# Haian-Jin/TensoIR

Hardware: AMD Instinct MI355X
Metric: primary+secondary rays/sec at 4096 rays x 512 samples (higher is better)
Workload: dtype f32 io and field; decoders split-bf16 x3 (hi/lo operands, 3 MFMA products), fp32 accumulate; indirect light (secondary-ray records): fp16 shadow taps + fp16 single-product decoder, fp32 accumulate

## Files before the change

### include/tensoir_hip.h

```cpp
#ifndef TENSOIR_HIP_H
#define TENSOIR_HIP_H

#include <stdint.h>

#ifdef __cplusplus
extern "C" {
#endif

#define TIR_VERSION 100

#define TIR_OK               0
#define TIR_ERR_ARG         -1001
#define TIR_ERR_UNSUPPORTED -1002
#define TIR_ERR_NO_DEVICE   -1003

typedef struct TirField {
    float aabb_min[3];
    float aabb_max[3];
    float inv_aabb[3];
    int32_t grid[3];
    float step_size;
    float distance_scale;
    float density_shift;
    float weight_thres;
    float near_, far_;
    int32_t act;
    int32_t n_dcomp;
    int32_t n_acomp;
    int32_t app_dim;
    int32_t n_lights;
    const float* dplane[3];
    const float* dline[3];
    const float* aplane[3];
    const float* aline[3];
    const float* basis_t;
    const float* light_line;
    const float* light_mean;
    const uint8_t* occ_nbr;
    int32_t occ_dim[3];
    float occ_aabb_min[3];
    float occ_inv[3];
    float occ_lo[3];
    float occ_hi[3];
    int32_t tune_lds_lines;
    int32_t tune_xcd_order;
    const float* dense_sigma;
    int32_t dense_pitch;
} TirField;

typedef struct TirFieldHalf {
    const void* aplane[3];
    const void* aline[3];
} TirFieldHalf;

#define TIR_HALF_MAX_JOBS 8
typedef struct TirHalfJob { const float* src; void* dst; int64_t n; unsigned* absmax; } TirHalfJob;
typedef struct TirHalfJobs { TirHalfJob job[TIR_HALF_MAX_JOBS]; } TirHalfJobs;

typedef struct TirMlp {
    const float* packed;
    int32_t feat_dim;
    int32_t pe;
    int32_t hidden;
    int32_t out_dim;
    int32_t act;
    int32_t tune_grid;
} TirMlp;

typedef struct TirEnvSG {
    const float* sgs;
    const float* rot;
    int32_t n_sg;
    int32_t n_lights;
} TirEnvSG;

int  tir_version(void);
const char* tir_error_string(int code);
int  tir_device_check(void);

int tir_pack_plane(const float* src, float* dst, int32_t C, int32_t H, int32_t W, void* stream);
int tir_pack_occupancy(const float* vol, uint8_t* nbr, int32_t W, int32_t H, int32_t D, void* stream);
int tir_pack_basis(const float* w, float* dst, int32_t app_dim, int32_t n_in, void* stream);
int tir_light_mean(const float* light_line, float* mean, int32_t L, int32_t n, void* stream);
int64_t tir_mlp_packed_floats(int32_t feat_dim, int32_t pe, int32_t hidden, int32_t out_dim);
int tir_pack_mlp(const float* w0, const float* b0, const float* w1, const float* b1,
                 const float* w2, const float* b2, int32_t feat_dim, int32_t pe, int32_t hidden,
                 int32_t out_dim, float* packed, void* stream);

int tir_vm_density_fwd(const TirField* f, const float* xyz, float* feat, float* sigma,
                       int64_t n, void* stream);

int tir_occupancy_query(const TirField* f, const float* xyz, uint8_t* hit, int64_t n, void* stream);

int tir_dense_alpha(const TirField* f, const float* lin_x, const float* lin_y, const float* lin_z,
                    int32_t gx, int32_t gy, int32_t gz, float length, float* alpha, void* stream);
int tir_alpha_pool(const float* alpha, int32_t gx, int32_t gy, int32_t gz, float thres, float* vol,
                   int32_t* bbox, void* stream);
int tir_filter_rays(const TirField* f, const float* rays, int64_t n, int32_t n_samples, int32_t bbox_only,
                    uint8_t* mask, void* stream);

int tir_dense_sigma_build(const TirField* f, float* vol, int32_t pitch, void* stream);
int tir_dense_sigma_fwd(const TirField* f, const float* xyz, float* feat, float* sigma, int64_t n, void* stream);

int tir_density_grad_fwd(const TirField* f, const float* xyz, float* sigma, float* grad,
                         float* normal, int64_t n, const int32_t* n_dev, void* stream);
int tir_density_feat_grad_fwd(const TirField* f, const float* xyz, float* feat, float* grad, int64_t n, void* stream);

int tir_vm_app_fwd(const TirField* f, const float* xyz, const int32_t* light_idx,
                   const int32_t* idx_map, float* rad_feat, float* int_feat, int32_t out_stride,
                   int32_t idx_div, int64_t n, const int32_t* n_dev, void* stream);

int tir_vm_app_jitter_fwd(const TirField* f, const float* xyz, int64_t n, const int32_t* n_dev, float scale,
                          uint64_t seed, uint64_t offset, const int64_t* rng_state, float* xyz_out,
                          float* int_feat, int32_t out_stride, void* stream);

int tir_vm_app_primary_fwd(const TirField* f, const float* xyz, const int32_t* light_idx, const int32_t* idx_map,
                           float* rad_feat, float* int_feat, int32_t out_stride, int64_t n, const int32_t* n_dev,
                           float scale, uint64_t seed, uint64_t offset, const int64_t* rng_state, float* xyz_out,
                           float* int_feat_jit, void* stream);
int tir_vm_app_primary_x3_fwd(const TirField* f, const float* xyz, const int32_t* light_idx, const int32_t* idx_map,
                              float* rad_feat, float* int_feat, int32_t out_stride, int64_t n, const int32_t* n_dev,
                              float scale, uint64_t seed, uint64_t offset, const int64_t* rng_state, float* xyz_out,
                              float* int_feat_jit, void* stream);
int tir_vm_app_fwd_x3(const TirField* f, const float* xyz, const int32_t* light_idx,
                      const int32_t* idx_map, float* rad_feat, float* int_feat, int32_t out_stride,
                      int32_t idx_div, int64_t n, const int32_t* n_dev, void* stream);
int tir_vm_app_fwd_bf16x3(const TirField* f, const float* xyz, const int32_t* light_idx,
                          const int32_t* idx_map, float* rad_feat, float* int_feat, int32_t out_stride,
                          int32_t idx_div, int64_t n, const int32_t* n_dev, void* stream);
int tir_vm_app_fwd_valu(const TirField* f, const float* xyz, const int32_t* light_idx,
                        const int32_t* idx_map, float* rad_feat, float* int_feat, int32_t out_stride,
                        int32_t idx_div, int64_t n, const int32_t* n_dev, void* stream);

int tir_mlp_fwd(const TirMlp* m, const float* feat, int32_t feat_stride, const float* aux,
                const int32_t* aux_map, int32_t aux_mod, float* out, int64_t n, const int32_t* n_dev,
        void* stream);
int tir_mlp_fwd_bf16x3(const TirMlp* m, const float* feat, int32_t feat_stride, const float* aux,
                       const int32_t* aux_map, int32_t aux_mod, float* out, int64_t n, const int32_t* n_dev,
        void* stream);

int tir_pack_half(const float* const* srcs, void* const* dsts, const int64_t* counts, int32_t n_tables, void* stream);
int tir_pack_half_checked(const float* const* srcs, void* const* dsts, const int64_t* counts, int32_t n_tables, float* absmax,
                          void* stream);
int tir_vm_app_fwd_h16(const TirField* f, const TirFieldHalf* fh, const float* xyz, const int32_t* light_idx,
                       const int32_t* idx_map, float* rad_feat, int32_t out_stride, int32_t idx_div, int64_t n,
                       const int32_t* n_dev, void* stream);

int tir_indirect_fused_fwd(const TirField* f, const TirFieldHalf* fh, const TirMlp* m, const float* xyz,
                           const int32_t* light_idx, const int32_t* rec_map, int32_t idx_div, int32_t aux_mod,
                           const float* table, float* out, int64_t n, const int32_t* n_dev, void* stream);

int tir_indirect_fused_hp_fwd(const TirField* f, const TirMlp* m, const float* xyz, const int32_t* light_idx,
                              const int32_t* rec_map, int32_t idx_div, int32_t aux_mod, const float* table, float* out,
                              int64_t n, const int32_t* n_dev, void* stream);

int tir_mlp_fwd_multi_bf16x3(const TirMlp* const* mlps, const float* const* feats, int32_t feat_stride,
                             const float* const* auxs, const int32_t* const* aux_maps, float* const* outs,
                             int32_t n_jobs, int64_t n, const int32_t* n_dev, void* stream);

int tir_mlp_aux_table(const TirMlp* m, const float* aux, int64_t n_aux, float* table, void* stream);
int tir_mlp_fwd_auxtab_bf16x3(const TirMlp* m, const float* feat, int32_t feat_stride, const float* table,
                              const int32_t* aux_map, int32_t aux_mod, float* out, int64_t n, const int32_t* n_dev,
                              void* stream);
int tir_mlp_fwd_auxtab_f16(const TirMlp* m, const float* feat, int32_t feat_stride, const float* table,
                           const int32_t* aux_map, int32_t aux_mod, float* out, int64_t n, const int32_t* n_dev,
                           void* stream);
int tir_mlp_train_fwd_auxtab_bf16x3(const TirMlp* m, const float* feat, int32_t feat_stride, const float* table,
                                    const int32_t* aux_map, int32_t aux_mod, float* out, float* h1, float* h2, int64_t n,
                                    const int32_t* n_dev, void* stream);
int tir_mlp_fwd_multi_auxtab_bf16x3(const TirMlp* const* mlps, const float* const* feats, int32_t feat_stride,
                                    const float* const* auxs, const int32_t* const* aux_maps,
                                    const float* const* tables, float* const* outs, int32_t n_jobs, int64_t n,
                                    const int32_t* n_dev, void* stream);
int tir_mlp_train_fwd_multi_bf16x3(const TirMlp* const* mlps, const float* const* feats, int32_t feat_stride,
                                   const float* const* auxs, const int32_t* const* aux_maps, float* const* outs,
                                   float* const* h1s, float* const* h2s, int32_t n_jobs, int64_t n,
                                   const int32_t* n_dev, void* stream);
int tir_mlp_fwd_bf16(const TirMlp* m, const float* feat, int32_t feat_stride, const float* aux,
                     const int32_t* aux_map, int32_t aux_mod, float* out, int64_t n, const int32_t* n_dev,
        void* stream);
int tir_mlp_fwd_valu(const TirMlp* m, const float* feat, int32_t feat_stride, const float* aux,
                     const int32_t* aux_map, int32_t aux_mod, float* out, int64_t n, const int32_t* n_dev,
        void* stream);

int tir_march_primary_fwd(const TirField* f, const float* rays, const float* ray_jitter,
// ... 360 lines not shown
```

### tensoir_amd/_lib.py

```python
from __future__ import annotations

import ctypes as C
import os

_HERE = os.path.dirname(os.path.abspath(__file__))
LIB_PATH = os.environ.get("TENSOIR_HIP_LIB", os.path.join(_HERE, "libtensoir_hip.so"))

c_float_p = C.c_void_p
c_int_p = C.c_void_p


class TirField(C.Structure):
    _fields_ = [
        ("aabb_min", C.c_float * 3), ("aabb_max", C.c_float * 3), ("inv_aabb", C.c_float * 3),
        ("grid", C.c_int32 * 3),
        ("step_size", C.c_float), ("distance_scale", C.c_float), ("density_shift", C.c_float),
        ("weight_thres", C.c_float), ("near_", C.c_float), ("far_", C.c_float),
        ("act", C.c_int32), ("n_dcomp", C.c_int32), ("n_acomp", C.c_int32), ("app_dim", C.c_int32),
        ("n_lights", C.c_int32),
        ("dplane", C.c_void_p * 3), ("dline", C.c_void_p * 3),
        ("aplane", C.c_void_p * 3), ("aline", C.c_void_p * 3),
        ("basis_t", C.c_void_p), ("light_line", C.c_void_p), ("light_mean", C.c_void_p),
        ("occ_nbr", C.c_void_p),
        ("occ_dim", C.c_int32 * 3), ("occ_aabb_min", C.c_float * 3), ("occ_inv", C.c_float * 3),
        ("occ_lo", C.c_float * 3), ("occ_hi", C.c_float * 3),
        ("tune_lds_lines", C.c_int32), ("tune_xcd_order", C.c_int32),
        ("dense_sigma", C.c_void_p), ("dense_pitch", C.c_int32),
    ]


class TirFieldHalf(C.Structure):
    _fields_ = [("aplane", C.c_void_p * 3), ("aline", C.c_void_p * 3)]


class TirFieldGrad(C.Structure):
    _fields_ = [("dplane", C.c_void_p * 3), ("dline", C.c_void_p * 3), ("aplane", C.c_void_p * 3),
                ("aline", C.c_void_p * 3), ("light_line", C.c_void_p), ("light_mean", C.c_void_p)]


class TirMlp(C.Structure):
    _fields_ = [("packed", C.c_void_p), ("feat_dim", C.c_int32), ("pe", C.c_int32),
                ("hidden", C.c_int32), ("out_dim", C.c_int32), ("act", C.c_int32), ("tune_grid", C.c_int32)]


class TirEnvSG(C.Structure):
    _fields_ = [("sgs", C.c_void_p), ("rot", C.c_void_p), ("n_sg", C.c_int32), ("n_lights", C.c_int32)]


P = C.c_void_p
I32 = C.c_int32
I64 = C.c_int64
F32 = C.c_float

SIGNATURES = {
    "tir_version": (C.c_int, []),
    "tir_error_string": (C.c_char_p, [C.c_int]),
    "tir_device_check": (C.c_int, []),
    "tir_pack_plane": (C.c_int, [P, P, I32, I32, I32, P]),
    "tir_pack_occupancy": (C.c_int, [P, P, I32, I32, I32, P]),
    "tir_pack_basis": (C.c_int, [P, P, I32, I32, P]),
    "tir_light_mean": (C.c_int, [P, P, I32, I32, P]),
    "tir_mlp_packed_floats": (I64, [I32, I32, I32, I32]),
    "tir_pack_mlp": (C.c_int, [P, P, P, P, P, P, I32, I32, I32, I32, P, P]),
    "tir_vm_density_fwd": (C.c_int, [C.POINTER(TirField), P, P, P, I64, P]),
    "tir_occupancy_query": (C.c_int, [C.POINTER(TirField), P, P, I64, P]),
    "tir_dense_alpha": (C.c_int, [C.POINTER(TirField), P, P, P, I32, I32, I32, F32, P, P]),
    "tir_alpha_pool": (C.c_int, [P, I32, I32, I32, F32, P, P, P]),
    "tir_filter_rays": (C.c_int, [C.POINTER(TirField), P, I64, I32, I32, P, P]),
    "tir_dense_sigma_build": (C.c_int, [C.POINTER(TirField), P, I32, P]),
    "tir_dense_sigma_fwd": (C.c_int, [C.POINTER(TirField), P, P, P, I64, P]),
    "tir_density_grad_fwd": (C.c_int, [C.POINTER(TirField), P, P, P, P, I64, P, P]),
    "tir_density_feat_grad_fwd": (C.c_int, [C.POINTER(TirField), P, P, P, I64, P]),
    "tir_vm_app_fwd": (C.c_int, [C.POINTER(TirField), P, P, P, P, P, I32, I32, I64, P, P]),
    "tir_vm_app_fwd_bf16x3": (C.c_int, [C.POINTER(TirField), P, P, P, P, P, I32, I32, I64, P, P]),
    "tir_vm_app_fwd_x3": (C.c_int, [C.POINTER(TirField), P, P, P, P, P, I32, I32, I64, P, P]),
    "tir_pack_half": (C.c_int, [P, P, P, I32, P]),
    "tir_pack_half_checked": (C.c_int, [P, P, P, I32, P, P]),
    "tir_vm_app_fwd_h16": (C.c_int, [C.POINTER(TirField), C.POINTER(TirFieldHalf), P, P, P, P, I32, I32, I64, P, P]),
    "tir_indirect_fused_fwd": (C.c_int, [C.POINTER(TirField), C.POINTER(TirFieldHalf), C.POINTER(TirMlp), P, P, P, I32, I32, P, P, I64, P, P]),
    "tir_indirect_fused_hp_fwd": (C.c_int, [C.POINTER(TirField), C.POINTER(TirMlp), P, P, P, I32, I32, P, P, I64, P, P]),
    "tir_vm_app_fwd_valu": (C.c_int, [C.POINTER(TirField), P, P, P, P, P, I32, I32, I64, P, P]),
    "tir_mlp_fwd": (C.c_int, [C.POINTER(TirMlp), P, I32, P, P, I32, P, I64, P, P]),
    "tir_mlp_fwd_bf16x3": (C.c_int, [C.POINTER(TirMlp), P, I32, P, P, I32, P, I64, P, P]),
    "tir_mlp_fwd_multi_bf16x3": (C.c_int, [P, P, I32, P, P, P, I32, I64, P, P]),
    "tir_mlp_fwd_multi_auxtab_bf16x3": (C.c_int, [P, P, I32, P, P, P, P, I32, I64, P, P]),
    "tir_mlp_aux_table": (C.c_int, [C.POINTER(TirMlp), P, I64, P, P]),
    "tir_mlp_fwd_auxtab_bf16x3": (C.c_int, [C.POINTER(TirMlp), P, I32, P, P, I32, P, I64, P, P]),
    "tir_mlp_fwd_auxtab_f16": (C.c_int, [C.POINTER(TirMlp), P, I32, P, P, I32, P, I64, P, P]),
    "tir_mlp_train_fwd_auxtab_bf16x3": (C.c_int, [C.POINTER(TirMlp), P, I32, P, P, I32, P, P, P, I64, P, P]),
    "tir_mlp_train_fwd_multi_bf16x3": (C.c_int, [P, P, I32, P, P, P, P, P, I32, I64, P, P]),
    "tir_mlp_fwd_bf16": (C.c_int, [C.POINTER(TirMlp), P, I32, P, P, I32, P, I64, P, P]),
    "tir_mlp_fwd_valu": (C.c_int, [C.POINTER(TirMlp), P, I32, P, P, I32, P, I64, P, P]),
    "tir_march_primary_fwd": (C.c_int, [C.POINTER(TirField), P, P, I32, I32, F32, P, P, P, P, P, P, P]),
    "tir_exclusive_scan": (C.c_int, [P, P, I32, P]),
    "tir_exclusive_scan_capped": (C.c_int, [P, P, I32, I32, P, P]),
    "tir_march_primary_fused_fwd": (C.c_int, [C.POINTER(TirField), P, P, I32, I32, F32, P, P, P, P, P, P,
                                              P, P, I32, P, P, I32, P, P]),
    "tir_composite_primary_fused": (C.c_int, [P, P, P, P, P, P, P, P, P, P, I32, I32, I32, F32, P, P, P, P, I64, P]),
    "tir_vm_app_jitter_fwd": (C.c_int, [C.POINTER(TirField), P, I64, P, F32, C.c_uint64, C.c_uint64, P, P, P, I32, P]),
    "tir_vm_app_primary_fwd": (C.c_int, [C.POINTER(TirField), P, P, P, P, P, I32, I64, P, F32, C.c_uint64, C.c_uint64, P, P, P, P]),
    "tir_vm_app_primary_x3_fwd": (C.c_int, [C.POINTER(TirField), P, P, P, P, P, I32, I64, P, F32, C.c_uint64, C.c_uint64, P, P, P, P]),
    "tir_compact_primary": (C.c_int, [C.POINTER(TirField), P, P, P, P, I32, I32, P, P, P, P, P]),
    "tir_composite_primary": (C.c_int, [P, P, P, P, P, P, P, P, P, P, I32, I32, I32, F32, P, P]),
    "tir_march_secondary_fwd": (C.c_int, [C.POINTER(TirField), P, P, P, P, P, I64, I32, I32, P, F32, P, P,
                                          P, I64, P, P, P, P, P, P, P]),
    "tir_accumulate_records": (C.c_int, [P, P, P, P, I64, P, P]),
    "tir_env_sg_fwd": (C.c_int, [C.POINTER(TirEnvSG), P, I32, P, P]),
    "tir_env_pixel_fwd": (C.c_int, [P, I32, I32, P, P, I32, I64, I32, P, P]),
    "tir_env_pixel_bwd": (C.c_int, [P, I32, I32, P, P, I32, I64, P, P, P]),
    "tir_shade_setup": (C.c_int, [P, P, P, I32, I32, F32, P, P, P]),
    "tir_shade_integrate": (C.c_int, [P, P, P, P, P, P, P, P, I32, I32, I32, I32, I32, F32, P, P]),
    "tir_shade_integrate_records": (C.c_int, [P, P, P, P, P, P, P, P, P, P, P, I32, I32, I32, I32, I32, F32, P, P, P]),
    "tir_shade_setup_compact": (C.c_int, [P, P, P, I32, I32, F32, P, P, P, P, P, P, I32, P]),
    "tir_march_secondary_ids_fwd": (C.c_int, [C.POINTER(TirField), P, P, P, P, P, I64, I32, I32, P, F32, P, P,
                                              P, I64, P, P, P, P, P, P, P, P, P]),
    "tir_relight_importance": (C.c_int, [P, P, P, P, P, P, P, P, P, I32, I32, P, P]),
    "tir_env_sample_setup": (C.c_int, [P, P, I32, I32, P, P, I32, I32, C.c_uint64, C.c_uint64, P, P, P]),
    "tir_env_sample_setup_list": (C.c_int, [P, P, I32, I32, P, I32, P, I32, I32, C.c_uint64, C.c_uint64, I32, I32, I32, P, P, I32, I32, P, P, P, P, P]),
    "tir_relight_importance_cells": (C.c_int, [P, P, P, P, P, P, P, P, P, P, I32, I32, P, P]),
    "tir_relight_importance_cells_packed": (C.c_int, [P, P, P, P, P, P, P, P, I32, I32, P, P]),
    "tir_env_lookup": (C.c_int, [P, I32, I32, P, I64, P, P]),
    "tir_surface_compact": (C.c_int, [P, P, I32, C.c_float, P, P, P, P, P, P, P, P, P]),
    "tir_env_sample_setup_list_n": (C.c_int, [P, P, I32, I32, P, I32, P, I32, I32, C.c_uint64, C.c_uint64, I32, I32, I32, P, P, I32, I32, P, P, P, P, P, P]),
    "tir_relight_importance_cells_packed_n": (C.c_int, [P, P, P, P, P, P, P, P, I32, I32, P, P, P]),
    "tir_env_compose": (C.c_int, [P, I32, I32, P, I32, I64, P, P, P, I32, P]),
    "tir_env_mis_setup": (C.c_int, [P, P, I32, I32, P, I32, P, P, P, P, P, I32, I32, I32, F32, C.c_uint64, C.c_uint64, I32, P, P, I32, I32,
                                    P, P, P, P, P, P, P, P]),
    "tir_relight_mis": (C.c_int, [P, P, P, P, P, P, P, P, P, P, I32, I32, I32, P, P, P]),
    "tir_ggx_specular": (C.c_int, [P, P, P, P, P, I32, I32, P, P]),
    "tir_march_primary_train_fwd": (C.c_int, [C.POINTER(TirField), P, P, I32, I32, F32, P, P, P, P, P, P, P]),
    "tir_composite_primary_bwd": (C.c_int, [P] * 11 + [I32, I32, I32, I32, F32] + [P] * 9 + [P]),
    "tir_march_primary_bwd": (C.c_int, [C.POINTER(TirField), C.POINTER(TirFieldGrad), P, P, I32, I32, P, P, P, P, P, P, P]),
    "tir_density_grad_bwd": (C.c_int, [C.POINTER(TirField), C.POINTER(TirFieldGrad), P, P, I64, P]),
    "tir_vm_density_bwd": (C.c_int, [C.POINTER(TirField), C.POINTER(TirFieldGrad), P, P, I64, P]),
    "tir_density_feat_bwd": (C.c_int, [C.POINTER(TirField), C.POINTER(TirFieldGrad), P, P, P, I64, P]),
    "tir_density_feat_grad_bwd": (C.c_int, [C.POINTER(TirField), C.POINTER(TirFieldGrad), P, P, P, I64, P]),
    "tir_vm_app_bwd": (C.c_int, [C.POINTER(TirField), C.POINTER(TirFieldGrad), P, P, P, P, P, I32, I64, P, P, P]),
    "tir_mlp_train_fwd": (C.c_int, [C.POINTER(TirMlp), P, I32, P, P, I32, P, P, P, I64, P, P]),
    "tir_mlp_train_fwd_bf16x3": (C.c_int, [C.POINTER(TirMlp), P, I32, P, P, I32, P, P, P, I64, P, P]),
    "tir_mlp_inputs": (C.c_int, [C.POINTER(TirMlp), P, I32, P, P, I32, P, I64, P]),
    "tir_mlp_bwd_packed_floats": (I64, [I32, I32, I32, I32]),
    "tir_pack_mlp_bwd": (C.c_int, [P, P, P, I32, I32, I32, I32, P, P]),
    "tir_mlp_bwd": (C.c_int, [C.POINTER(TirMlp), P, P, I32, P, P, P, P, I64, P, P, P, P, P]),
    "tir_mlp_bwd_bf16x3": (C.c_int, [C.POINTER(TirMlp), P, P, I32, P, P, P, P, I64, P, P, P, P, P]),
    "tir_mlp_bwd_multi_bf16x3": (C.c_int, [P, P, P, I32, P, P, P, P, I32, I64, P, P, P, P, P]),
    "tir_gemm_tn_small_bf16x3": (C.c_int, [P, I32, I32, P, I32, I32, I32, I64, P, I32, P]),
    "tir_mlp_wgrad_multi": (C.c_int, [P, P, P, P, P, P, I32, P, P, P, P, P, P, P, P, I32, I64, I32, P]),
    "tir_record_check": (C.c_int, [P, P, I32, P, P, P]),
    "tir_adam_step": (C.c_int, [I32, P, P, P, P, P, P, P, P, F32, F32, F32, P]),
    "tir_gemm_tn": (C.c_int, [P, I32, I32, P, I32, I32, I32, I64, P, I32, P, P]),
    "tir_gemm_tn_bf16x3": (C.c_int, [P, I32, I32, P, I32, I32, I32, I64, P, I32, P, P]),
    "tir_shade_integrate_bwd": (C.c_int, [P, P, P, P, P, P, P, P, I32, I32, I32, I32, I32, F32, P, P, P, P]),
    "tir_env_sg_bwd": (C.c_int, [C.POINTER(TirEnvSG), P, I32, P, P, P]),
# ... 73 lines not shown
```

### tensoir_amd/csrc/tir_common.hpp

```cpp
#pragma once
#include <hip/hip_runtime.h>
#include <stdint.h>
#include <initializer_list>
#include <type_traits>
#include "tensoir_hip.h"

#define TIR_WAVE 64

#define TIR_CHECK_LAUNCH()                                   \
    do {                                                     \
        hipError_t e__ = hipGetLastError();                  \
        if (e__ != hipSuccess) return -(int)e__;             \
    } while (0)

static inline hipStream_t tir_stream(void* s) { return reinterpret_cast<hipStream_t>(s); }

static inline int tir_xcd_mapping(const TirField* f) { return f->tune_xcd_order == 1 ? 1 : 0; }

#include <mutex>
#include <set>
#include <utility>
static inline int tir_allow_dynamic_lds(const void* kernel, int bytes) {
    static std::mutex mu;
    static std::set<std::pair<const void*, int>> done;
    int dev = 0;
    hipError_t e = hipGetDevice(&dev);
    if (e != hipSuccess) return -(int)e;
    std::lock_guard<std::mutex> lock(mu);
    if (done.count({kernel, dev})) return TIR_OK;
    e = hipFuncSetAttribute(kernel, hipFuncAttributeMaxDynamicSharedMemorySize, bytes);
    if (e != hipSuccess) return -(int)e;
    done.insert({kernel, dev});
    return TIR_OK;
}

static inline bool tir_occ_index_ok(const TirField* f) {
    if (!f->occ_nbr) return true;
    const int64_t W = f->occ_dim[0], H = f->occ_dim[1], D = f->occ_dim[2];
    return W > 0 && H > 0 && D > 0 && W + 1 < (1 << 24) && (H + 1) * (D + 1) < (1 << 24) && (W + 1) * (H + 1) * (D + 1) < ((int64_t)1 << 31);
}

static inline bool tir_plane_index_ok(const TirField* f) {
    for (int i = 0; i < 3; ++i)
        for (int j = i + 1; j < 3; ++j)
            if ((int64_t)f->grid[i] * f->grid[j] * f->n_dcomp * 4 >= ((int64_t)1 << 32) || (int64_t)f->grid[i] * f->n_dcomp * 4 >= (1 << 24) || (int64_t)f->grid[j] * f->n_dcomp * 4 >= (1 << 24)) return false;
    return true;
}

static inline bool tir_app_index_ok(const TirField* f) {
    for (int i = 0; i < 3; ++i)
        for (int j = i + 1; j < 3; ++j)
            if ((int64_t)f->grid[i] * f->grid[j] * f->n_acomp >= ((int64_t)1 << 31)) return false;
    for (int i = 0; i < 3; ++i)
        if ((int64_t)f->grid[i] * f->n_acomp >= (1 << 24)) return false;
    return true;
}

static inline bool tir_dense_sigma_ok(const TirField* f) {
    if (!f->dense_sigma || f->dense_pitch <= f->grid[0]) return false;
    const int64_t Y = f->grid[1], Z = f->grid[2], pb = (int64_t)f->dense_pitch * 4;
    return f->grid[0] >= 2 && Y >= 1 && Z >= 1 && Y * Z < (1 << 24) && pb < (1 << 24) && Y * Z * pb < ((int64_t)1 << 32);
}

static inline bool tir_any_null(std::initializer_list<const void*> ptrs) {
    for (const void* p : ptrs) if (!p) return true;
    return false;
}
static inline bool tir_aligned16(std::initializer_list<const void*> ptrs) {
    for (const void* p : ptrs) if (reinterpret_cast<uintptr_t>(p) % 16 != 0) return false;
    return true;
}

struct TirAppNeeds {
    const TirFieldHalf* half = nullptr;
    bool aligned16 = false;
    bool light_mean = true;
    bool index32 = false;
    int n_acomp = 0;
    int app_dim = 0;
    bool feature_rows = true;
    int stride_max = 32;
    TirAppNeeds& fp16_tables(const TirFieldHalf* fh) { half = fh; return *this; }
    TirAppNeeds& aligned() { aligned16 = true; return *this; }
    TirAppNeeds& no_light_mean() { light_mean = false; return *this; }
    TirAppNeeds& element_index32() { index32 = true; return *this; }
    TirAppNeeds& width(int n) { n_acomp = n; return *this; }
    TirAppNeeds& app_dim_is(int d) { app_dim = d; return *this; }
    TirAppNeeds& no_feature_rows() { feature_rows = false; return *this; }
    TirAppNeeds& stride_unbounded() { stride_max = 0x7fffffff; return *this; }
};

static inline int tir_check_app_field(const TirField* f, const TirAppNeeds& need, int out_stride) {
    for (int i = 0; i < 3; ++i) {
        const void* plane = need.half ? need.half->aplane[i] : static_cast<const void*>(f->aplane[i]);
        const void* line = need.half ? need.half->aline[i] : static_cast<const void*>(f->aline[i]);
        if (f->grid[i] < 2 || !plane || !line || (need.aligned16 && !tir_aligned16({plane, line}))) return TIR_ERR_ARG;
    }
    if (!f->basis_t || !f->light_line || (need.light_mean && !f->light_mean)) return TIR_ERR_ARG;
    if (need.n_acomp && f->n_acomp != need.n_acomp) return TIR_ERR_UNSUPPORTED;
    if (need.app_dim ? f->app_dim != need.app_dim : (f->app_dim < 1 || f->app_dim > 27)) return TIR_ERR_UNSUPPORTED;
    if (need.index32 && !tir_app_index_ok(f)) return TIR_ERR_UNSUPPORTED;
    if (need.feature_rows && (out_stride < f->app_dim || out_stride > need.stride_max)) return TIR_ERR_ARG;
    return TIR_OK;
}

template <typename Go>
static inline int tir_with_rows(int64_t n, std::initializer_list<const void*> need, std::initializer_list<const void*> aligned, Go&& go) {
    if (n < 0 || (n > 0 && tir_any_null(need)) || !tir_aligned16(aligned)) return TIR_ERR_ARG;
    if (n == 0) return TIR_OK;
    return go();
}

constexpr int TIR_APP_LDS_LIMIT = 160 * 1024;

static inline unsigned tir_gather_blocks(int64_t n, int rows, int cap, int xcd_on) {
    int64_t blocks = (n + rows - 1) / rows;
    if (blocks > cap) blocks = cap;
    if (xcd_on) blocks = (blocks + 7) / 8 * 8;
    return (unsigned)blocks;
}

static inline unsigned tir_job_split(int64_t units, int total, int n_jobs) {
    int per = total / n_jobs;
    if (per < 1) per = 1;
    if (units < per) per = (int)units;
    return (unsigned)(per * n_jobs);
}

template <typename... P, typename... A>
static inline int tir_launch(void (*kernel)(P...), int lds_limit, dim3 grid, dim3 block, size_t lds, hipStream_t s, const A&... args) {
    if (lds_limit > 0)
        if (int rc = tir_allow_dynamic_lds(reinterpret_cast<const void*>(kernel), lds_limit)) return rc;
    hipLaunchKernelGGL(kernel, grid, block, lds, s, args...);
    TIR_CHECK_LAUNCH();
    return TIR_OK;
}

template <int... C4S, typename Fn>
static inline int tir_dispatch_c4(int n_acomp, Fn&& fn) {
    int rc = TIR_ERR_UNSUPPORTED;
    (void)((n_acomp == 4 * C4S && ((rc = fn(std::integral_constant<int, C4S>{})), true)) || ...);
    return rc;
}

// ... 354 lines not shown
__device__ __forceinline__ float scan_prod(float v, int ) {
    v *= dpp_f<0x111, 0xf>(1.0f, v);
    v *= dpp_f<0x112, 0xf>(1.0f, v);
    v *= dpp_f<0x114, 0xf>(1.0f, v);
    v *= dpp_f<0x118, 0xf>(1.0f, v);
    v *= dpp_f<0x142, 0xa>(1.0f, v);
    if (WIDTH == 64) v *= dpp_f<0x143, 0xc>(1.0f, v);
    return v;
}

template <int WIDTH>
__device__ __forceinline__ float shift_up1(float incl, int lane_in_group) {
    float o = dpp_f<0x138, 0xf>(1.0f, incl);
    return lane_in_group == 0 ? 1.0f : o;
}

template <int WIDTH>
__device__ __forceinline__ float group_sum(float v) {
#pragma unroll
    for (int d = WIDTH / 2; d > 0; d >>= 1) v += __shfl_xor(v, d, WIDTH);
    return v;
}

template <int C4>
__device__ __forceinline__ float wave_sigma_t(const TirField& f, bool valid, float x, float y, float z, float* wl) {
    const int lane = threadIdx.x & 63;
    const unsigned long long m = __ballot(valid);
    const int n = __popcll(m);
    if (n == 0) return 0.0f;
    const int rank = __popcll(m & ((1ull << lane) - 1ull));
    if (valid) { wl[rank * 4] = x; wl[rank * 4 + 1] = y; wl[rank * 4 + 2] = z; }
    __builtin_amdgcn_wave_barrier();
    constexpr int PER = 64 / C4;
    const int slot_in = lane / C4, c = lane % C4;
    for (int base = 0; base < n; base += PER) {
        const int slot = base + slot_in;
        float part = 0.0f;
        if (slot < n) {
            const float4 p = *reinterpret_cast<const float4*>(wl + slot * 4);
            part = density_feature_chunk<C4>(f, p.x, p.y, p.z, c);
        }
        if (C4 >= 2) part += dpp_f<0xB1, 0xf>(0.0f, part);
        if (C4 >= 4) part += dpp_f<0x4E, 0xf>(0.0f, part);
        if (C4 >= 8) part += dpp_f<0x141, 0xf>(0.0f, part);
        if (slot < n && c == 0) wl[slot * 4 + 3] = part;
    }
    __builtin_amdgcn_wave_barrier();
    float sig = 0.0f;
    if (valid) sig = feature2density(f, wl[rank * 4 + 3]);
    __builtin_amdgcn_wave_barrier();
    return sig;
}

#define TIR_TAPREC 9

__device__ __forceinline__ unsigned mad_u24(unsigned a, unsigned b, unsigned c) {
    unsigned r;
    asm("v_mad_u32_u24 %0, %1, %2, %3" : "=v"(r) : "v"(a), "v"(b), "v"(c));
    return r;
}

typedef float tir_f2u __attribute__((ext_vector_type(2), aligned(4)));

__device__ __forceinline__ tir_f2 ld2b(const float* base, unsigned byte_off) {
    const tir_f2u v = *reinterpret_cast<const tir_f2u*>(reinterpret_cast<const char*>(base) + byte_off);
    return tir_f2{v.x, v.y};
}

__device__ __forceinline__ float dense_feature(const TirField& f, float x, float y, float z) {
    const TapQ tx = make_tap_q(x, f.grid[0]), ty = make_tap_q(y, f.grid[1]), tz = make_tap_q(z, f.grid[2]);
    const bool below = tx.i1 == 0u;
    const float wx0 = below ? tx.w.y : tx.w.x, wx1 = below ? 0.0f : tx.w.y;
    const unsigned pb = (unsigned)f.dense_pitch * 4u, xo = tx.i0 * 4u;
    const unsigned z0 = mul_u24(tz.i0, (unsigned)f.grid[1]), z1 = mul_u24(tz.i1, (unsigned)f.grid[1]);
    const tir_f2 v00 = ld2b(f.dense_sigma, mad_u24(z0 + ty.i0, pb, xo));
    const tir_f2 v01 = ld2b(f.dense_sigma, mad_u24(z0 + ty.i1, pb, xo));
    const tir_f2 v10 = ld2b(f.dense_sigma, mad_u24(z1 + ty.i0, pb, xo));
    const tir_f2 v11 = ld2b(f.dense_sigma, mad_u24(z1 + ty.i1, pb, xo));
    const float a = fmaf(v00.y, wx1, v00.x * wx0), b = fmaf(v01.y, wx1, v01.x * wx0);
    const float c = fmaf(v10.y, wx1, v10.x * wx0), d = fmaf(v11.y, wx1, v11.x * wx0);
    const float e = fmaf(b, ty.w.y, a * ty.w.x), g = fmaf(d, ty.w.y, c * ty.w.x);
    return fmaf(g, tz.w.y, e * tz.w.x);
}
__device__ __forceinline__ unsigned lds_addr(const float* p) {
#if defined(__HIP_DEVICE_COMPILE__)
    return (unsigned)(uintptr_t)(const __attribute__((address_space(3))) float*)p;
#else
    return 0;
#endif
}
__device__ __forceinline__ float4 lds_ld4(unsigned addr) {
#if defined(__HIP_DEVICE_COMPILE__)
    return *(const __attribute__((address_space(3))) float4*)(uintptr_t)addr;
#else
    return float4{};
#endif
}

template <int C4>
__device__ __forceinline__ float density_chunk_rec(const TirField& f, const float* __restrict__ ll, const unsigned* __restrict__ rec, int c) {
    constexpr unsigned TB = C4 * 16;
    const unsigned pk[3] = {rec[0], rec[1], rec[2]};
    unsigned ix[3][2];
#pragma unroll
    for (int a = 0; a < 3; ++a) { ix[a][0] = pk[a] & 0xffffu; ix[a][1] = pk[a] >> 16; }
    const unsigned cb = 16u * (unsigned)c;
    unsigned col[2][2];
#pragma unroll
    for (int a = 0; a < 2; ++a) { col[a][0] = mad_u24(ix[a][0], TB, cb); col[a][1] = mad_u24(ix[a][1], TB, cb); }
    float acc = 0.0f;
    unsigned laddr = lds_addr(ll) + cb;
#pragma unroll
    for (int i = 0; i < 3; ++i) {
        const int m0 = (i == 2) ? 1 : 0, m1 = (i == 0) ? 1 : 2, vi = 2 - i;
        const unsigned row_bytes = (unsigned)f.grid[m0] * TB;
        const float* pl = f.dplane[i];
        const float4 a = ld4b(pl, mad_u24(ix[m1][0], row_bytes, col[m0][0]));
        const float4 b = ld4b(pl, mad_u24(ix[m1][0], row_bytes, col[m0][1]));
        const float4 cc = ld4b(pl, mad_u24(ix[m1][1], row_bytes, col[m0][0]));
        const float4 d = ld4b(pl, mad_u24(ix[m1][1], row_bytes, col[m0][1]));
        const float4 e = lds_ld4(mad_u24(ix[vi][0], TB, laddr));
        const float4 g = lds_ld4(mad_u24(ix[vi][1], TB, laddr));
        laddr += (unsigned)f.grid[vi] * TB;
        const tir_f2 w0 = {__uint_as_float(rec[3 + 2 * m0]), __uint_as_float(rec[4 + 2 * m0])};
        const tir_f2 w1 = {__uint_as_float(rec[3 + 2 * m1]), __uint_as_float(rec[4 + 2 * m1])};
        const tir_f2 wv = {__uint_as_float(rec[3 + 2 * vi]), __uint_as_float(rec[4 + 2 * vi])};
        const tir_f2 wa = w0 * tir_f2{w1.x, w1.x}, wb = w0 * tir_f2{w1.y, w1.y};
        acc = plane_line_4ch(a, b, cc, d, e, g, wa, wb, wv, acc);
    }
    return acc;
}

template <int C4>
__device__ __forceinline__ float wave_sigma_lds(const TirField& f, const float* __restrict__ ll, bool valid, float x, float y,
                                                float z, float* wl) {
    const int lane = threadIdx.x & 63;
    const unsigned long long m = __ballot(valid);
    const int n = __popcll(m);
    if (n == 0) return 0.0f;
    const int rank = __popcll(m & ((1ull << lane) - 1ull));
    unsigned* const wr = reinterpret_cast<unsigned*>(wl);
    if (valid) {
        const TapQ tx = make_tap_q(x, f.grid[0]), ty = make_tap_q(y, f.grid[1]), tz = make_tap_q(z, f.grid[2]);
        unsigned* r = wr + rank * TIR_TAPREC;
        r[0] = tx.i0 | (tx.i1 << 16); r[1] = ty.i0 | (ty.i1 << 16); r[2] = tz.i0 | (tz.i1 << 16);
        r[3] = __float_as_uint(tx.w.x); r[4] = __float_as_uint(tx.w.y);
        r[5] = __float_as_uint(ty.w.x); r[6] = __float_as_uint(ty.w.y);
        r[7] = __float_as_uint(tz.w.x); r[8] = __float_as_uint(tz.w.y);
    }
    __builtin_amdgcn_wave_barrier();
    constexpr int PER = 64 / C4;
    const int slot_in = lane / C4, c = lane % C4;
    for (int base = 0; base < n; base += PER) {
        const int slot = base + slot_in;
        float part = 0.0f;
        if (slot < n) part = density_chunk_rec<C4>(f, ll, wr + slot * TIR_TAPREC, c);
        if (C4 >= 2) part += dpp_f<0xB1, 0xf>(0.0f, part);
        if (C4 >= 4) part += dpp_f<0x4E, 0xf>(0.0f, part);
        if (C4 >= 8) part += dpp_f<0x141, 0xf>(0.0f, part);
        if (slot < n && c == 0) wl[slot * TIR_TAPREC] = part;
    }
    __builtin_amdgcn_wave_barrier();
    float sig = 0.0f;
    if (valid) sig = feature2density(f, wl[rank * TIR_TAPREC]);
    __builtin_amdgcn_wave_barrier();
    return sig;
// ... 192 lines not shown
```

### tensoir_amd/csrc/tir_field.hip

```cpp
#include "tir_common.hpp"

using namespace tir;

__global__ void k_pack_plane(const float* __restrict__ src, float* __restrict__ dst, int C, int HW) {
    int64_t i = (int64_t)blockIdx.x * blockDim.x + threadIdx.x;
    if (i >= (int64_t)C * HW) return;
    int c = (int)(i % C);
    int64_t t = i / C;
    dst[i] = src[(int64_t)c * HW + t];
}

__global__ void k_pack_occ(const float* __restrict__ vol, uint8_t* __restrict__ nbr, int W, int H, int D) {
    int64_t i = (int64_t)blockIdx.x * blockDim.x + threadIdx.x;
    const int64_t n = (int64_t)(W + 1) * (H + 1) * (D + 1);
    if (i >= n) return;
    const int x0 = (int)(i % (W + 1)) - 1, y0 = (int)((i / (W + 1)) % (H + 1)) - 1, z0 = (int)(i / ((int64_t)(W + 1) * (H + 1))) - 1;
    uint32_t m = 0;
    for (int c = 0; c < 8; ++c) {
        const int xx = x0 + (c & 1), yy = y0 + ((c >> 1) & 1), zz = z0 + (c >> 2);
        if (xx >= 0 && xx < W && yy >= 0 && yy < H && zz >= 0 && zz < D && vol[((int64_t)zz * H + yy) * W + xx] > 0.5f) m |= 1u << c;
    }
    nbr[i] = (uint8_t)m;
}

// ... 1118 lines not shown
    return tir_with_rows(n, {xyz}, {}, [&] {
        constexpr int C4 = 12, CA = 48;
        const int lt_rows = f->n_lights <= 16 ? f->n_lights : 0;
        const size_t w_floats = HX ? (2 * 3 * 2 * 2 * 64 * 16) / 4 : 3 * CA * 32;
        const size_t x_floats = HX ? (2 * 2 * 16 * TIR_XHX * 2) / 4 : 2 * CA * TIR_XLD;
        const int nb = (int)tir_gather_blocks(n, 64, 1024, 1);
        const dim3 g(2 * nb), b(256);
        const int xcd_on = tir_xcd_mapping(f);
        const TirJitter jt{scale, (unsigned long long)seed, (unsigned long long)offset, reinterpret_cast<const long long*>(rng_state), xyz_out};
        if (f->n_lights == 1) {
            const size_t lds1 = (w_floats + (size_t)2 * 3 * CA + 4 * (x_floats / 2)) * sizeof(float);
            return tir_launch(k_vm_app_primary_one<C4, HX>, TIR_APP_LDS_LIMIT, g, b, lds1, tir_stream(stream), *f, xyz, rad_feat, int_feat,
                              int_feat_jit, out_stride, n, n_dev, xcd_on, jt, nb);
        }
        const size_t lds = (w_floats + (size_t)(lt_rows + 1) * 3 * CA + 4 * x_floats) * sizeof(float);
        return tir_launch(k_vm_app_primary<C4, HX>, TIR_APP_LDS_LIMIT, g, b, lds, tir_stream(stream), *f, xyz, light_idx, idx_map, rad_feat,
                          int_feat, int_feat_jit, out_stride, n, n_dev, xcd_on, jt, lt_rows, nb);
    });
}

extern "C" int tir_vm_app_primary_fwd(const TirField* f, const float* xyz, const int32_t* light_idx, const int32_t* idx_map,
                                      float* rad_feat, float* int_feat, int32_t out_stride, int64_t n, const int32_t* n_dev,
                                      float scale, uint64_t seed, uint64_t offset, const int64_t* rng_state, float* xyz_out,
                                      float* int_feat_jit, void* stream) {
    return app_primary_fwd<false>(f, xyz, light_idx, idx_map, rad_feat, int_feat, out_stride, n, n_dev, scale, seed, offset, rng_state,
                                  xyz_out, int_feat_jit, stream);
}

extern "C" int tir_vm_app_primary_x3_fwd(const TirField* f, const float* xyz, const int32_t* light_idx, const int32_t* idx_map,
                                         float* rad_feat, float* int_feat, int32_t out_stride, int64_t n, const int32_t* n_dev,
                                         float scale, uint64_t seed, uint64_t offset, const int64_t* rng_state, float* xyz_out,
                                         float* int_feat_jit, void* stream) {
    return app_primary_fwd<true>(f, xyz, light_idx, idx_map, rad_feat, int_feat, out_stride, n, n_dev, scale, seed, offset, rng_state,
                                 xyz_out, int_feat_jit, stream);
}

extern "C" int tir_vm_app_fwd_x3(const TirField* f, const float* xyz, const int32_t* light_idx,
                                 const int32_t* idx_map, float* rad_feat, float* int_feat, int32_t out_stride,
                                 int32_t idx_div, int64_t n, const int32_t* n_dev, void* stream) {
    return app_fwd(f, xyz, light_idx, idx_map, rad_feat, int_feat, out_stride, idx_div, n, n_dev, stream, APP_HX);
}

extern "C" int tir_vm_app_fwd_valu(const TirField* f, const float* xyz, const int32_t* light_idx,
                                   const int32_t* idx_map, float* rad_feat, float* int_feat, int32_t out_stride,
                                   int32_t idx_div, int64_t n, const int32_t* n_dev, void* stream) {
    return app_fwd(f, xyz, light_idx, idx_map, rad_feat, int_feat, out_stride, idx_div, n, n_dev, stream, APP_VALU);
}

extern "C" int tir_vm_app_fwd_bf16x3(const TirField* f, const float* xyz, const int32_t* light_idx,
                                     const int32_t* idx_map, float* rad_feat, float* int_feat, int32_t out_stride,
                                     int32_t idx_div, int64_t n, const int32_t* n_dev, void* stream) {
    return app_fwd(f, xyz, light_idx, idx_map, rad_feat, int_feat, out_stride, idx_div, n, n_dev, stream, APP_BF16X3);
}

static int pack_half_launch(const float* const* srcs, void* const* dsts, const int64_t* counts, int32_t n_tables, float* absmax, void* stream) {
    if (n_tables < 0 || n_tables > TIR_HALF_MAX_JOBS || (n_tables > 0 && (!srcs || !dsts || !counts))) return TIR_ERR_ARG;
    if (n_tables == 0) return TIR_OK;
    TirHalfJobs jobs;
    int64_t most = 0;
    for (int i = 0; i < n_tables; ++i) {
        if (counts[i] < 0 || (counts[i] > 0 && !srcs[i])) return TIR_ERR_ARG;
        if (counts[i] > 0 && !dsts[i] && !absmax) return TIR_ERR_ARG;
        if (reinterpret_cast<uintptr_t>(srcs[i]) % 16 != 0 || reinterpret_cast<uintptr_t>(dsts[i]) % 16 != 0) return TIR_ERR_ARG;
        jobs.job[i] = TirHalfJob{srcs[i], dsts[i], counts[i], absmax ? reinterpret_cast<unsigned*>(absmax) + i : nullptr};
        most = counts[i] > most ? counts[i] : most;
    }
    if (most == 0) return TIR_OK;
    const int64_t per_block = 2048 * TIR_PACK_CHUNKS;
    hipLaunchKernelGGL(k_pack_half, dim3((unsigned)((most + per_block - 1) / per_block), (unsigned)n_tables), dim3(256), 0, tir_stream(stream), jobs);
    TIR_CHECK_LAUNCH();
    return TIR_OK;
}

extern "C" int tir_pack_half(const float* const* srcs, void* const* dsts, const int64_t* counts, int32_t n_tables, void* stream) {
    return pack_half_launch(srcs, dsts, counts, n_tables, nullptr, stream);
}

extern "C" int tir_pack_half_checked(const float* const* srcs, void* const* dsts, const int64_t* counts, int32_t n_tables, float* absmax,
                                     void* stream) {
    if (!absmax) return TIR_ERR_ARG;
    return pack_half_launch(srcs, dsts, counts, n_tables, absmax, stream);
}

extern "C" int tir_vm_app_fwd_h16(const TirField* f, const TirFieldHalf* fh, const float* xyz, const int32_t* light_idx,
                                  const int32_t* idx_map, float* rad_feat, int32_t out_stride, int32_t idx_div, int64_t n,
                                  const int32_t* n_dev, void* stream) {
    if (!f || !fh) return TIR_ERR_ARG;
    if (int rc = tir_check_app_field(f, TirAppNeeds().fp16_tables(fh).aligned().element_index32().width(48), out_stride)) return rc;
    return tir_with_rows(n, {xyz, rad_feat, light_idx}, {}, [&] {
        const int lt_rows = f->n_lights <= 16 ? f->n_lights : 0;
        const size_t lds = (size_t)(3 * 3 * 2 * 32) * 16 + (size_t)(lt_rows + 1) * 144 * sizeof(float) + (size_t)4 * 32 * TIR_XH * 2;
        const int xcd_on = tir_xcd_mapping(f);
        return tir_launch(k_vm_app_h16, 0, dim3(tir_gather_blocks(n, 128, 2048, xcd_on)), dim3(256), lds, tir_stream(stream), *f, *fh, xyz,
                          light_idx, idx_map, rad_feat, out_stride, idx_div, n, n_dev, xcd_on, lt_rows);
    });
}
```

### tensoir_amd/csrc/tir_mlp.hip

```cpp
#include "tir_common.hpp"

typedef float f32x16 __attribute__((ext_vector_type(16)));
typedef float f32x4 __attribute__((ext_vector_type(4)));

namespace {

constexpr int F = 27;
constexpr int PE = 2;
constexpr int HID = 128;
constexpr int IN = F + 3 + 2 * PE * F + 2 * PE * 3;
constexpr int HALF = IN / 2;
constexpr int NPF = PE * F;
constexpr int R0 = HALF - NPF;

constexpr int OFF_W0 = 0;
constexpr int OFF_B0 = OFF_W0 + IN * HID;
constexpr int OFF_W1 = OFF_B0 + HID;
constexpr int OFF_B1 = OFF_W1 + HID * HID;
constexpr int OFF_W2 = OFF_B1 + HID;
constexpr int OFF_B2 = OFF_W2 + 2 * 64 * 4;
constexpr int MFMA_FLOATS = OFF_B2 + 4;
constexpr int OFF_RW0 = MFMA_FLOATS;
constexpr int OFF_RB0 = OFF_RW0 + HID * IN;
constexpr int OFF_RW1 = OFF_RB0 + HID;
// ... 659 lines not shown

__device__ __forceinline__ int fus_feature_of_row(int row) {
    const int kg = (row >> 2) & 1, slot = (row >> 3) * 4 + (row & 3);
    if (kg == 0) return slot < FUS_NF0 ? slot : -1;
    return slot < F - FUS_NF0 ? FUS_NF0 + slot : -1;
}

template <int KK>
__device__ __forceinline__ float fus_input(const float (&fo)[16]) {
    constexpr int j = KK / 5, kind = KK % 5;
    if constexpr (j >= FUS_NF0) return 0.0f;
    else if constexpr (kind == 4) return fo[j];
    else {
        const float c_hi = 0.15915493667125702f, c_lo = 6.4206382432985265e-09f;
        const float kr = rintf(fo[j] * c_hi);
        float t = fmaf(fo[j], c_hi, -kr);
        t = fmaf(fo[j], c_lo, t);
        const float sn = __builtin_amdgcn_sinf(t), cs = __builtin_amdgcn_sinf(t + 0.25f);
        if constexpr (kind == 0) return sn;
        else if constexpr (kind == 1) return (sn + sn) * cs;
        else if constexpr (kind == 2) return cs;
        else return fmaf(-(sn + sn), sn, 1.0f);
    }
}

template <int KB>
__device__ __forceinline__ void fus_layer1(unsigned whi, const float (&fo)[16], f32x16 (&acc)[4]) {
    bf16x8 ah[4], al[4];
#pragma unroll
    for (int mt = 0; mt < 4; ++mt) ah[mt] = lds_tile(whi, KB * 4096 + mt * 512);
    const float v[8] = {fus_input<KB * 8 + 0>(fo), fus_input<KB * 8 + 1>(fo), fus_input<KB * 8 + 2>(fo), fus_input<KB * 8 + 3>(fo),
                        fus_input<KB * 8 + 4>(fo), fus_input<KB * 8 + 5>(fo), fus_input<KB * 8 + 6>(fo), fus_input<KB * 8 + 7>(fo)};
    bf16x8 xh, xl = {};
    cvt8_f16(v, xh);
    mfma12<1, true>(ah, al, xh, xl, acc);
    __builtin_amdgcn_sched_barrier(0);
    if constexpr (KB + 1 < KB0A) fus_layer1<KB + 1>(whi, fo, acc);
}

typedef _Float16 fus_f16x2 __attribute__((ext_vector_type(2)));

template <int KB>
__device__ __forceinline__ void fus_layer2p(unsigned whi, const unsigned (&hp)[32], f32x16 (&acc)[4]) {
    bf16x8 ah[4], al[4];
#pragma unroll
    for (int mt = 0; mt < 4; ++mt) ah[mt] = lds_tile(whi, KB * 4096 + mt * 512);
    const u32x4_t H = {hp[4 * KB], hp[4 * KB + 1], hp[4 * KB + 2], hp[4 * KB + 3]};
    const bf16x8 xh = __builtin_bit_cast(bf16x8, H), xl = {};
    mfma12<1, true>(ah, al, xh, xl, acc);
    __builtin_amdgcn_sched_barrier(0);
    if constexpr (KB + 1 < KB1) fus_layer2p<KB + 1>(whi, hp, acc);
}

struct FusGroup { unsigned o00, o01, o10, o11, l0, l1; tir::tir_h2 w00, w01, w10, w11, wl0, wl1; };

__device__ __forceinline__ FusGroup fus_group(const TirField& f, const tir::TapQ (&ax)[3], const unsigned (&xb)[3][2], const int k) {
    constexpr int CA = 48;
    const int m0 = (k == 2) ? 1 : 0, m1 = (k == 0) ? 1 : 2, vi = 2 - k;
    const tir::TapQ &tx = ax[m0], &ty = ax[m1], &tl = ax[vi];
    FusGroup g;
    const float w00 = tx.w.x * ty.w.x, w01 = tx.w.y * ty.w.x, w10 = tx.w.x * ty.w.y, w11 = tx.w.y * ty.w.y;
    g.w00 = tir::tir_h2{(_Float16)w00, (_Float16)w00}; g.w01 = tir::tir_h2{(_Float16)w01, (_Float16)w01};
    g.w10 = tir::tir_h2{(_Float16)w10, (_Float16)w10}; g.w11 = tir::tir_h2{(_Float16)w11, (_Float16)w11};
    g.wl0 = tir::tir_h2{(_Float16)tl.w.x, (_Float16)tl.w.x}; g.wl1 = tir::tir_h2{(_Float16)tl.w.y, (_Float16)tl.w.y};
    const unsigned row_bytes = (unsigned)f.grid[m0] * (2 * CA);
    const unsigned r0 = tir::mul_u24(ty.i0, row_bytes), r1 = tir::mul_u24(ty.i1, row_bytes);
    g.o00 = r0 + xb[m0][0]; g.o01 = r0 + xb[m0][1]; g.o10 = r1 + xb[m0][0]; g.o11 = r1 + xb[m0][1];
    g.l0 = xb[vi][0]; g.l1 = xb[vi][1];
    return g;
}

struct FusChunk { uint4 a, b, c, d, e, g; };

__device__ __forceinline__ uint4 ld_u4b(const void* base, unsigned byte_off) {
    return *reinterpret_cast<const uint4*>(reinterpret_cast<const char*>(base) + byte_off);
}

__device__ __forceinline__ void fus_issue(FusChunk& c, const void* __restrict__ pl, const void* __restrict__ ln, const FusGroup& g, const int q) {
    const unsigned o = 32u * (unsigned)q;
    c.a = ld_u4b(pl, g.o00 + o); c.b = ld_u4b(pl, g.o01 + o); c.c = ld_u4b(pl, g.o10 + o); c.d = ld_u4b(pl, g.o11 + o);
    c.e = ld_u4b(ln, g.l0 + o);  c.g = ld_u4b(ln, g.l1 + o);
}

template <int NW, bool PACK>
__global__ void __launch_bounds__(NW * 64)
k_indirect_fused(TirField f, TirFieldHalf fh, const float* __restrict__ packed, const float* __restrict__ xyz,
                 const int32_t* __restrict__ light_idx, const int32_t* __restrict__ rec_map, int idx_div, int aux_mod,
                 const float* __restrict__ table, float* __restrict__ out, int64_t n, const int32_t* __restrict__ n_dev,
                 int out_dim, int act, int lt_rows) {
    using namespace tir;
    constexpr int CA = 48;
    extern __shared__ __attribute__((aligned(16))) float lds[];
    for (int i = threadIdx.x * 4; i < FH_FLOATS; i += NW * 64 * 4)
        *reinterpret_cast<float4*>(lds + i) = *reinterpret_cast<const float4*>(packed + OFF_FF + i);
    f16x8* Wh = reinterpret_cast<f16x8*>(lds + FH_FLOATS);
    float* LT = lds + FH_FLOATS + FUS_WH_BYTES / 4;
    const int n_lt = lt_rows;
    const int lane = threadIdx.x & 63, wave = threadIdx.x >> 6;
    _Float16* X = reinterpret_cast<_Float16*>(LT + (n_lt + 1) * (3 * CA)) + wave * (32 * FUS_XH);
    for (int e = threadIdx.x; e < 3 * 3 * 2 * 32; e += NW * 64) {
        const int row = e & 31, kg = (e >> 5) & 1, t = (e >> 6) % 3, k = e / 192;
        const int feat = fus_feature_of_row(row);
        f16x8 hv;
#pragma unroll
        for (int q = 0; q < 8; ++q) hv[q] = feat >= 0 ? sat_half(f.basis_t[(size_t)(k * CA + 16 * t + 8 * kg + q) * 32 + feat]) : (_Float16)0.0f;
        Wh[e] = hv;
    }
    _Float16* LT16 = reinterpret_cast<_Float16*>(LT);
    for (int i = threadIdx.x; i < n_lt * 3 * CA; i += NW * 64) LT16[i] = sat_half(f.light_line[i]);
    for (int i = threadIdx.x * 4; i < 3 * CA; i += NW * 64 * 4)
        *reinterpret_cast<float4*>(LT + n_lt * 3 * CA + i) = *reinterpret_cast<const float4*>(f.light_mean + i);
    __syncthreads();
    if (n_dev) n = min(n, (int64_t)max(*n_dev, 0));
    const int sl = lane & 31, h = lane >> 5;
    const int gj = lane >> 1, gc = lane & 1;
    const unsigned lds0 = (unsigned)(size_t)lds;
    const unsigned lane_off = lds0 + BH_FLOATS * 4 + (unsigned)(h * 128 + sl) * 16;
    const unsigned w0hi = opaque(lane_off);
    const unsigned w1hi = opaque(lane_off + BW0A_ELEMS * 2);
    constexpr int TILE = NW * 32;
    const int64_t n_tiles = (n + TILE - 1) / TILE;
    const UDiv by_div = make_udiv(idx_div), by_mod = make_udiv(aux_mod);
    for (int64_t tile = blockIdx.x; tile < n_tiles; tile += gridDim.x) {
        const int64_t r0 = tile * TILE + wave * 32;
        const int64_t sg = r0 + gj, sgc = sg < n ? sg : n - 1;
        const float p[3] = {xyz[3 * sgc], xyz[3 * sgc + 1], xyz[3 * sgc + 2]};
        const float* lrow;
        const _Float16* lrow16;
        {
            int li = 0;
            if (f.n_lights > 1) {
                unsigned lsel = rec_map ? (unsigned)rec_map[sgc] : (unsigned)sgc, rem_;
                lsel = udiv(lsel, by_div, rem_);
                li = light_idx[lsel];
                li = min(max(li, 0), f.n_lights - 1);
            }
            lrow = n_lt ? LT + li * (3 * CA) : f.light_line + (size_t)li * (3 * CA);
            lrow16 = LT16 + li * (3 * CA);
        }
        const int64_t sd = r0 + sl, sdc = sd < n ? sd : n - 1;
        unsigned ai = rec_map ? (unsigned)rec_map[sdc] : (unsigned)sdc;
        if (aux_mod > 0) udiv(ai, by_mod, ai);
        f32x16 facc;
#pragma unroll
        for (int r = 0; r < 16; ++r) facc[r] = 0.0f;
        f32x16 acc[4];
        auto load_table = [&]() {
            const float* tp = table + (size_t)ai * HID + 4 * h;
#pragma unroll
            for (int mt = 0; mt < 4; ++mt)
#pragma unroll
                for (int i = 0; i < 4; ++i) {
                    const float4 t4 = *reinterpret_cast<const float4*>(tp + mt * 32 + 8 * i);
                    acc[mt][4 * i] = t4.x; acc[mt][4 * i + 1] = t4.y; acc[mt][4 * i + 2] = t4.z; acc[mt][4 * i + 3] = t4.w;
                }
        };
        {
            TapQ ax[3];
            unsigned xb[3][2];
#pragma unroll
            for (int a = 0; a < 3; ++a) {
                ax[a] = make_tap_q(p[a], f.grid[a]);
                xb[a][0] = mul_u24(ax[a].i0, 2 * CA) + 16u * (unsigned)gc;
                xb[a][1] = mul_u24(ax[a].i1, 2 * CA) + 16u * (unsigned)gc;
            }
            FusGroup G[3];
            FusChunk ck[3];
            G[0] = fus_group(f, ax, xb, 0);
            fus_issue(ck[0], fh.aplane[0], fh.aline[0], G[0], 0);
            fus_issue(ck[1], fh.aplane[0], fh.aline[0], G[0], 1);
            fus_issue(ck[2], fh.aplane[0], fh.aline[0], G[0], 2);
#pragma unroll
            for (int i = 0; i < 9; ++i) {
                const int k = i / 3, q = i % 3;
                FusChunk& c = ck[i % 3];
                const int ch0 = 16 * q + 8 * gc;
                *reinterpret_cast<uint4*>(X + gj * FUS_XH + ch0) =
                    h16_chunk_pk(c.a, c.b, c.c, c.d, c.e, c.g, G[k].w00, G[k].w01, G[k].w10, G[k].w11, G[k].wl0, G[k].wl1,
                                 n_lt ? *reinterpret_cast<const uint4*>(lrow16 + k * CA + ch0) : pack8_half(lrow + k * CA + ch0));
                if (i + 3 < 9) {
                    const int k2 = (i + 3) / 3, q2 = (i + 3) % 3;
                    if (q2 == 0) G[k2] = fus_group(f, ax, xb, k2);
                    fus_issue(c, fh.aplane[k2], fh.aline[k2], G[k2], q2);
                }
                __builtin_amdgcn_wave_barrier();
                const f16x8 a = Wh[((k * 3 + q) * 2 + h) * 32 + sl];
                const f16x8 b = *reinterpret_cast<const f16x8*>(X + sl * FUS_XH + 16 * q + 8 * h);
                facc = __builtin_amdgcn_mfma_f32_32x32x16_f16(a, b, facc, 0, 0, 0);
                __builtin_amdgcn_wave_barrier();
            }
        }
        __builtin_amdgcn_s_setprio(FUS_DECODER_PRIO);
        float fo[16];
#pragma unroll
        for (int r = 0; r < 16; ++r) fo[r] = __builtin_amdgcn_fmed3f(facc[r], -65504.0f, 65504.0f);
        if (PACK) load_table();
        fus_layer1<0>(w0hi, fo, acc);
        f32x16 acc2[4];
        if constexpr (PACK) {
            unsigned hp[32];
#pragma unroll
            for (int q = 0; q < 64; q += 2) {
                const f32x2_t v2 = {acc[q >> 4][q & 15], acc[(q + 1) >> 4][(q + 1) & 15]};
                fus_f16x2 hv = __builtin_convertvector(v2, fus_f16x2);
                hv = __builtin_elementwise_min(__builtin_elementwise_max(hv, fus_f16x2{(_Float16)0.0f, (_Float16)0.0f}),
                                               fus_f16x2{(_Float16)65504.0f, (_Float16)65504.0f});
                hp[q >> 1] = __builtin_bit_cast(unsigned, hv);
            }
#pragma unroll
            for (int mt = 0; mt < 4; ++mt) {
                const float* bp = lds + BH_B1 + (h * 4 + mt) * 16;
#pragma unroll
                for (int r = 0; r < 16; ++r) acc2[mt][r] = bp[r];
            }
            fus_layer2p<0>(w1hi, hp, acc2);
        } else {
#pragma unroll
            for (int mt = 0; mt < 4; ++mt) {
                const float* bp = lds + BH_B1 + (h * 4 + mt) * 16;
#pragma unroll
                for (int r = 0; r < 16; ++r) acc2[mt][r] = bp[r];
            }
            layer2_interleaved<1, 0, true>(w1hi, w1hi, acc, acc2);
        }
        f32x4 o4[4];
#pragma unroll
        for (int c = 0; c < 4; ++c) o4[c] = f32x4{0.f, 0.f, 0.f, 0.f};
        {
            const float* wp = lds + BH_W2 + (h * 4 + (lane & 3)) * W2A_STRIDE;
#pragma unroll
            for (int g = 0; g < 16; ++g) {
                const float4 w = *reinterpret_cast<const float4*>(wp + 4 * g);
                const float wv[4] = {w.x, w.y, w.z, w.w};
#pragma unroll
                for (int e = 0; e < 4; ++e) {
                    const int q = 4 * g + e;
                    const float x = acc2[q >> 4][q & 15];
                    o4[e] = __builtin_amdgcn_mfma_f32_4x4x1f32(wv[e], x + __builtin_fabsf(x), o4[e], 0, 0, 0);
                }
            }
        }
        float o0 = (o4[0][0] + o4[1][0]) + (o4[2][0] + o4[3][0]);
        float o1 = (o4[0][1] + o4[1][1]) + (o4[2][1] + o4[3][1]);
        float o2 = (o4[0][2] + o4[1][2]) + (o4[2][2] + o4[3][2]);
        float o3 = (o4[0][3] + o4[1][3]) + (o4[2][3] + o4[3][3]);
        o0 += __shfl_xor(o0, 32, 64); o1 += __shfl_xor(o1, 32, 64);
        o2 += __shfl_xor(o2, 32, 64); o3 += __shfl_xor(o3, 32, 64);
        __builtin_amdgcn_s_setprio(0);
        if (h == 0 && sd < n) {
            const float* b2 = lds + BH_B2;
            float* op = out + sd * out_dim;
            op[0] = act_out(o0 + b2[0], act);
            if (out_dim > 1) op[1] = act_out(o1 + b2[1], act);
            if (out_dim > 2) op[2] = act_out(o2 + b2[2], act);
            if (out_dim > 3) op[3] = act_out(o3 + b2[3], act);
        }
    }
}

constexpr int HP_XS = 24;
constexpr int HP_X_HALVES = 2 * 32 * HP_XS;

typedef __attribute__((address_space(3))) const long lds_i64;
__device__ __forceinline__ long lds_tile8(unsigned base, int byte_off) {
    return *reinterpret_cast<lds_i64*>(base + (unsigned)byte_off);
}

__device__ __forceinline__ long cvt8_fp8(const float (&c)[8]) {
    int lo = 0, hi = 0;
    lo = __builtin_amdgcn_cvt_pk_fp8_f32(c[0], c[1], lo, false);
    lo = __builtin_amdgcn_cvt_pk_fp8_f32(c[2], c[3], lo, true);
    hi = __builtin_amdgcn_cvt_pk_fp8_f32(c[4], c[5], hi, false);
    hi = __builtin_amdgcn_cvt_pk_fp8_f32(c[6], c[7], hi, true);
    return (long)(((unsigned long)(unsigned)hi << 32) | (unsigned long)(unsigned)lo);
}

template <int KK>
__device__ __forceinline__ float fus_input8(const float (&fo)[16], const float (&fo8)[16]) {
    if constexpr (KK % 5 == 4 && KK / 5 < FUS_NF0) return fo8[KK / 5];
    else return fus_input<KK>(fo);
}

typedef int hp_i32x8 __attribute__((ext_vector_type(8)));
typedef __attribute__((address_space(3))) const u32x4_t lds_u32x4;

__device__ __forceinline__ void hp_residue(unsigned w8, int byte_off, const hp_i32x8& xs, f32x16 (&acc)[4]) {
#pragma unroll
    for (int mt = 0; mt < 4; ++mt) {
        const u32x4_t lo = *reinterpret_cast<lds_u32x4*>(w8 + (unsigned)(byte_off + mt * 1024));
        const u32x4_t hi = *reinterpret_cast<lds_u32x4*>(w8 + (unsigned)(byte_off + mt * 1024 + 16));
        const hp_i32x8 a = {(int)lo[0], (int)lo[1], (int)lo[2], (int)lo[3], (int)hi[0], (int)hi[1], (int)hi[2], (int)hi[3]};
        acc[mt] = __builtin_amdgcn_mfma_scale_f32_32x32x64_f8f6f4(a, xs, acc[mt], 0, 0, 0, 110, 0, 127);
    }
}

template <int KB>
__device__ __forceinline__ void hp_layer1(unsigned whi, unsigned w8, const float (&fo)[16], const float (&fo8)[16], f32x16 (&acc)[4],
                                          hp_i32x8& xs) {
    bf16x8 ah[4];
#pragma unroll
    for (int mt = 0; mt < 4; ++mt) ah[mt] = lds_tile(whi, KB * 4096 + mt * 512);
    const float v[8] = {fus_input<KB * 8 + 0>(fo), fus_input<KB * 8 + 1>(fo), fus_input<KB * 8 + 2>(fo), fus_input<KB * 8 + 3>(fo),
                        fus_input<KB * 8 + 4>(fo), fus_input<KB * 8 + 5>(fo), fus_input<KB * 8 + 6>(fo), fus_input<KB * 8 + 7>(fo)};
    const float v8[8] = {fus_input8<KB * 8 + 0>(fo, fo8), fus_input8<KB * 8 + 1>(fo, fo8), fus_input8<KB * 8 + 2>(fo, fo8), fus_input8<KB * 8 + 3>(fo, fo8),
                         fus_input8<KB * 8 + 4>(fo, fo8), fus_input8<KB * 8 + 5>(fo, fo8), fus_input8<KB * 8 + 6>(fo, fo8), fus_input8<KB * 8 + 7>(fo, fo8)};
    bf16x8 xh;
    cvt8_f16(v, xh);
    const long x8 = cvt8_fp8(v8);
    if constexpr (KB % 4 == 0) xs = hp_i32x8{0, 0, 0, 0, 0, 0, 0, 0};
    xs[2 * (KB % 4)] = (int)(unsigned)(unsigned long)x8;
    xs[2 * (KB % 4) + 1] = (int)(unsigned)((unsigned long)x8 >> 32);
#pragma unroll
    for (int mt = 0; mt < 4; ++mt)
        acc[mt] = __builtin_amdgcn_mfma_f32_32x32x16_f16(__builtin_bit_cast(f16x8, ah[mt]), __builtin_bit_cast(f16x8, xh), acc[mt], 0, 0, 0);
    if constexpr (KB % 4 == 3 || KB + 1 == KB0A) hp_residue(w8, (KB / 4) * 8192, xs, acc);
    __builtin_amdgcn_sched_barrier(0);
    if constexpr (KB + 1 < KB0A) hp_layer1<KB + 1>(whi, w8, fo, fo8, acc, xs);
}

template <int KB>
__device__ __forceinline__ void hp_layer2(unsigned whi, unsigned w8, const unsigned (&hp)[32], const unsigned (&h8)[16], f32x16 (&acc)[4]) {
    bf16x8 ah[4];
#pragma unroll
    for (int mt = 0; mt < 4; ++mt) ah[mt] = lds_tile(whi, KB * 4096 + mt * 512);
    const u32x4_t H = {hp[4 * KB], hp[4 * KB + 1], hp[4 * KB + 2], hp[4 * KB + 3]};
#pragma unroll
    for (int mt = 0; mt < 4; ++mt)
        acc[mt] = __builtin_amdgcn_mfma_f32_32x32x16_f16(__builtin_bit_cast(f16x8, ah[mt]), __builtin_bit_cast(f16x8, H), acc[mt], 0, 0, 0);
    if constexpr (KB % 4 == 3) {
        constexpr int g = KB / 4;
        const hp_i32x8 xs = {(int)h8[8 * g], (int)h8[8 * g + 1], (int)h8[8 * g + 2], (int)h8[8 * g + 3],
                             (int)h8[8 * g + 4], (int)h8[8 * g + 5], (int)h8[8 * g + 6], (int)h8[8 * g + 7]};
        hp_residue(w8, g * 8192, xs, acc);
    }
    __builtin_amdgcn_sched_barrier(0);
    if constexpr (KB + 1 < KB1) hp_layer2<KB + 1>(whi, w8, hp, h8, acc);
}

constexpr unsigned HP_TB = 192;
// ... 1252 lines not shown
        if (SAVE && n > 0 && (!h1s[i] || !h2s[i])) return TIR_ERR_ARG;
        if (!tir_aligned16({feats[i], tab})) return TIR_ERR_ARG;
        jobs.j[i] = TirMlpJob{mlps[i]->packed, feats[i], auxs[i], aux_maps ? aux_maps[i] : nullptr, outs[i], mlps[i]->out_dim,
                              mlps[i]->act, SAVE ? h1s[i] : nullptr, SAVE ? h2s[i] : nullptr, tab};
    }
    if (n == 0) return TIR_OK;
    return tir_launch(k_mlp_bf16_multi<3, SAVE>, BF_BYTES, dim3(tir_job_split((n + 255) / 256, 256, n_jobs)), dim3(512), (size_t)BF_BYTES,
                      tir_stream(stream), jobs, feat_stride, n, n_dev);
}

extern "C" int tir_mlp_fwd_multi_bf16x3(const TirMlp* const* mlps, const float* const* feats, int32_t feat_stride,
                                        const float* const* auxs, const int32_t* const* aux_maps, float* const* outs,
                                        int32_t n_jobs, int64_t n, const int32_t* n_dev, void* stream) {
    return launch_multi<false>(mlps, feats, feat_stride, auxs, aux_maps, outs, nullptr, nullptr, n_jobs, n, n_dev, stream);
}

extern "C" int tir_mlp_fwd_multi_auxtab_bf16x3(const TirMlp* const* mlps, const float* const* feats, int32_t feat_stride,
                                               const float* const* auxs, const int32_t* const* aux_maps,
                                               const float* const* tables, float* const* outs, int32_t n_jobs, int64_t n,
                                               const int32_t* n_dev, void* stream) {
    return launch_multi<false>(mlps, feats, feat_stride, auxs, aux_maps, outs, nullptr, nullptr, n_jobs, n, n_dev, stream, tables);
}

extern "C" int tir_mlp_train_fwd_multi_bf16x3(const TirMlp* const* mlps, const float* const* feats, int32_t feat_stride,
                                              const float* const* auxs, const int32_t* const* aux_maps, float* const* outs,
                                              float* const* h1s, float* const* h2s, int32_t n_jobs, int64_t n,
                                              const int32_t* n_dev, void* stream) {
    return launch_multi<true>(mlps, feats, feat_stride, auxs, aux_maps, outs, h1s, h2s, n_jobs, n, n_dev, stream);
}

extern "C" int tir_mlp_aux_table(const TirMlp* m, const float* aux, int64_t n_aux, float* table, void* stream) {
    if (int rc = check_mlp(m)) return rc;
    return tir_with_rows(n_aux, {aux, table}, {}, [&] {
        return tir_launch(k_mlp_aux_table, 0, dim3((unsigned)((n_aux * HID + 255) / 256)), dim3(256), 0, tir_stream(stream), m->packed, aux,
                          n_aux, table);
    });
}

#define TIR_AUXT_ARGS m->packed, feat, feat_stride, table, aux_map, aux_mod, out, n, n_dev, m->out_dim, m->act
template <bool F16, bool SAVE>
static int mlp_fwd_auxtab(const TirMlp* m, const float* feat, int32_t feat_stride, const float* table, const int32_t* aux_map,
                          int32_t aux_mod, float* out, float* h1, float* h2, int64_t n, const int32_t* n_dev, void* stream) {
    const auto go = [&] {
        const bool vec = rows_vec(feat, feat_stride);
        const dim3 g(decoder_grid(n, 256, m->tune_grid)), b(512);
        hipStream_t s = tir_stream(stream);
        if constexpr (F16)
            return vec ? tir_launch(k_mlp_f16_auxt<true>, FH_BYTES, g, b, FH_BYTES, s, TIR_AUXT_ARGS)
                       : tir_launch(k_mlp_f16_auxt<false>, FH_BYTES, g, b, FH_BYTES, s, TIR_AUXT_ARGS);
        else
            return vec ? tir_launch(k_mlp_bf16_auxt<true, SAVE>, BFA_BYTES, g, b, BFA_BYTES, s, TIR_AUXT_ARGS, h1, h2)
                       : tir_launch(k_mlp_bf16_auxt<false, SAVE>, BFA_BYTES, g, b, BFA_BYTES, s, TIR_AUXT_ARGS, h1, h2);
    };
    if constexpr (SAVE) return with_decoder_rows(m, n, feat_stride, {}, {feat, table, out, h1, h2}, {table}, go);
    else return with_decoder_rows(m, n, feat_stride, {}, {feat, table, out}, {table}, go);
}

#undef TIR_AUXT_ARGS

extern "C" int tir_mlp_fwd_auxtab_bf16x3(const TirMlp* m, const float* feat, int32_t feat_stride, const float* table,
                                         const int32_t* aux_map, int32_t aux_mod, float* out, int64_t n, const int32_t* n_dev,
                                         void* stream) {
    return mlp_fwd_auxtab<false, false>(m, feat, feat_stride, table, aux_map, aux_mod, out, nullptr, nullptr, n, n_dev, stream);
}

extern "C" int tir_mlp_fwd_auxtab_f16(const TirMlp* m, const float* feat, int32_t feat_stride, const float* table,
                                      const int32_t* aux_map, int32_t aux_mod, float* out, int64_t n, const int32_t* n_dev,
                                      void* stream) {
    return mlp_fwd_auxtab<true, false>(m, feat, feat_stride, table, aux_map, aux_mod, out, nullptr, nullptr, n, n_dev, stream);
}

extern "C" int tir_mlp_train_fwd_auxtab_bf16x3(const TirMlp* m, const float* feat, int32_t feat_stride, const float* table,
                                               const int32_t* aux_map, int32_t aux_mod, float* out, float* h1, float* h2,
                                               int64_t n, const int32_t* n_dev, void* stream) {
    return mlp_fwd_auxtab<false, true>(m, feat, feat_stride, table, aux_map, aux_mod, out, h1, h2, n, n_dev, stream);
}

extern "C" int tir_indirect_fused_fwd(const TirField* f, const TirFieldHalf* fh, const TirMlp* m, const float* xyz,
                                      const int32_t* light_idx, const int32_t* rec_map, int32_t idx_div, int32_t aux_mod,
                                      const float* table, float* out, int64_t n, const int32_t* n_dev, void* stream) {
    if (!f || !fh) return TIR_ERR_ARG;
    if (int rc = check_mlp(m)) return rc;
    if (int rc = tir_check_app_field(f, TirAppNeeds().fp16_tables(fh).aligned().element_index32().width(48).app_dim_is(F).no_feature_rows(), 0)) return rc;
    return tir_with_rows(n, {xyz, light_idx, table, out}, {table}, [&] {
        if (!fused_index_ok(n, idx_div, aux_mod)) return (int)TIR_ERR_UNSUPPORTED;
        const int lt_rows = f->n_lights <= 16 ? f->n_lights : 0;
        constexpr int NW = 12; constexpr bool PACK = true;
        const size_t lds = (size_t)FH_BYTES + FUS_WH_BYTES + (size_t)(lt_rows + 1) * 144 * sizeof(float) + (size_t)NW * 32 * FUS_XH * 2;
        return tir_launch(k_indirect_fused<NW, PACK>, (int)lds, dim3(decoder_grid(n, NW * 32, m->tune_grid)), dim3(NW * 64), lds,
                          tir_stream(stream), *f, *fh, m->packed, xyz, light_idx, rec_map, idx_div, aux_mod, table, out, n, n_dev,
                          m->out_dim, m->act, lt_rows);
    });
}

extern "C" int tir_indirect_fused_hp_fwd(const TirField* f, const TirMlp* m, const float* xyz, const int32_t* light_idx,
                                         const int32_t* rec_map, int32_t idx_div, int32_t aux_mod, const float* table, float* out,
                                         int64_t n, const int32_t* n_dev, void* stream) {
    if (!f) return TIR_ERR_ARG;
    if (int rc = check_mlp(m)) return rc;
    if (int rc = tir_check_app_field(f, TirAppNeeds().aligned().no_light_mean().element_index32().width(48).app_dim_is(F).no_feature_rows(), 0)) return rc;
    for (int i = 0; i < 3; ++i)
        for (int j = i + 1; j < 3; ++j)
            if ((int64_t)f->grid[i] * HP_TB >= (1 << 24) || (int64_t)f->grid[j] * HP_TB >= (1 << 24) ||
                (int64_t)f->grid[i] * f->grid[j] * HP_TB >= ((int64_t)1 << 32)) return TIR_ERR_UNSUPPORTED;
    return tir_with_rows(n, {xyz, light_idx, table, out}, {table}, [&] {
        if (!fused_index_ok(n, idx_div, aux_mod)) return (int)TIR_ERR_UNSUPPORTED;
        if (f->n_lights < 1 || f->n_lights > 8) return (int)TIR_ERR_UNSUPPORTED;
        const int lt_rows = f->n_lights;
        constexpr int NW = 8;
        const size_t lds = (size_t)FH_BYTES + (size_t)F8_FLOATS * 4 + 2 * (size_t)FUS_WH_BYTES + (size_t)lt_rows * 144 * sizeof(float) +
                           (size_t)NW * HP_X_HALVES * 2;
        return tir_launch(k_indirect_fused_hp<NW>, (int)lds, dim3(decoder_grid(n, NW * 32, m->tune_grid)), dim3(NW * 64), lds,
                          tir_stream(stream), *f, m->packed, xyz, light_idx, rec_map, idx_div, aux_mod, table, out, n, n_dev, m->out_dim,
                          m->act, lt_rows);
    });
}

extern "C" int64_t tir_mlp_bwd_packed_floats(int32_t feat_dim, int32_t pe, int32_t hidden, int32_t out_dim) {
    return mlp_shape_built(feat_dim, pe, hidden, out_dim) ? (int64_t)BWD_TOTAL_FLOATS : (int64_t)TIR_ERR_UNSUPPORTED;
}

extern "C" int tir_pack_mlp_bwd(const float* w0, const float* w1, const float* w2, int32_t feat_dim, int32_t pe,
                                int32_t hidden, int32_t out_dim, float* packed, void* stream) {
    if (tir_any_null({w0, w1, w2, packed})) return TIR_ERR_ARG;
    if (!mlp_shape_built(feat_dim, pe, hidden, out_dim)) return TIR_ERR_UNSUPPORTED;
    return tir_launch(k_pack_mlp_bwd, 0, dim3((BWD_TOTAL_FLOATS + 255) / 256), dim3(256), 0, tir_stream(stream), w0, w1, w2, out_dim, packed);
}

template <typename Kernel>
static int mlp_bwd(Kernel kernel, size_t lds, const TirMlp* m, const float* packed_bwd, const float* feat, int32_t feat_stride,
                   const float* out, const float* g_out, const float* h1, const float* h2, int64_t n, float* g_feat, float* dz1,
                   float* dz2, float* dz3, void* stream) {
    return with_decoder_rows(m, n, feat_stride, {packed_bwd}, {feat, out, g_out, h1, h2, g_feat, dz1, dz2, dz3}, {}, [&] {
        return tir_launch(kernel, (int)lds, dim3(decoder_grid(n, 256, NO_TUNE_GRID)), dim3(512), lds, tir_stream(stream), packed_bwd, feat,
                          feat_stride, out, g_out, h1, h2, n, m->out_dim, m->act, g_feat, dz1, dz2, dz3);
    });
}

extern "C" int tir_mlp_bwd(const TirMlp* m, const float* packed_bwd, const float* feat, int32_t feat_stride,
                           const float* out, const float* g_out, const float* h1, const float* h2, int64_t n,
                           float* g_feat, float* dz1, float* dz2, float* dz3, void* stream) {
    return mlp_bwd(k_mlp_bwd, (size_t)BWD_FLOATS * sizeof(float), m, packed_bwd, feat, feat_stride, out, g_out, h1, h2, n, g_feat, dz1, dz2,
                   dz3, stream);
}

extern "C" int tir_mlp_bwd_bf16x3(const TirMlp* m, const float* packed_bwd, const float* feat, int32_t feat_stride,
                           const float* out, const float* g_out, const float* h1, const float* h2, int64_t n,
                           float* g_feat, float* dz1, float* dz2, float* dz3, void* stream) {
    return mlp_bwd(k_mlp_bwd_bf16, (size_t)BWD_BF_LDS_BYTES, m, packed_bwd, feat, feat_stride, out, g_out, h1, h2, n, g_feat, dz1, dz2, dz3,
                   stream);
}

extern "C" int tir_mlp_bwd_multi_bf16x3(const TirMlp* const* mlps, const float* const* packed_bwds, const float* const* feats,
                                       int32_t feat_stride, const float* const* outs, const float* const* g_outs,
                                       const float* const* h1s, const float* const* h2s, int32_t n_jobs, int64_t n,
                                       float* const* g_feats, float* const* dz1s, float* const* dz2s, float* const* dz3s, void* stream) {
    if (n_jobs < 1 || n_jobs > 4 || tir_any_null({mlps, packed_bwds, feats, outs, g_outs, h1s, h2s, g_feats, dz1s, dz2s, dz3s}) || n < 0 ||
        feat_stride < F)
        return TIR_ERR_ARG;
    TirMlpBwdJobs jobs;
    jobs.n_jobs = n_jobs;
    for (int i = 0; i < n_jobs; ++i) {
        if (int rc = check_mlp(mlps[i])) return rc;
        if (!packed_bwds[i]) return TIR_ERR_ARG;
        if (n > 0 && tir_any_null({feats[i], outs[i], g_outs[i], h1s[i], h2s[i], g_feats[i], dz1s[i], dz2s[i], dz3s[i]})) return TIR_ERR_ARG;
        jobs.j[i] = TirMlpBwdJob{packed_bwds[i], feats[i], outs[i], g_outs[i], h1s[i], h2s[i], g_feats[i], dz1s[i], dz2s[i], dz3s[i],
                                 mlps[i]->out_dim, mlps[i]->act};
    }
    if (n == 0) return TIR_OK;
    return tir_launch(k_mlp_bwd_bf16_multi, BWD_BF_LDS_BYTES, dim3(tir_job_split((n + 255) / 256, 256, n_jobs)), dim3(512),
// ... 30 lines not shown
```

### tensoir_amd/field_model.py

```python
from __future__ import annotations

import functools
import math
import time

import numpy as np
import torch
import torch.nn as nn
import torch.nn.functional as F

from . import capacity, indirect, ops, regularisers
from ._lib import TensoirHipError, TirField

MAT_MODE = [[0, 1], [0, 2], [1, 2]]
VEC_MODE = [2, 1, 0]


def raw2alpha(sigma, dist):
    alpha = 1.0 - torch.exp(-sigma * dist)
    T = torch.cumprod(torch.cat([torch.ones(alpha.shape[0], 1).to(alpha.device), 1.0 - alpha + 1e-10], -1), -1)
    weights = alpha * T[:, :-1]
    return alpha, weights, T[:, -1:]


# ... 468 lines not shown

    def TV_loss_app(self, reg):
        return regularisers.model_tv(self.app_plane, reg)

    def _field_params(self):
        d = self.__dict__["_parameters"], self.__dict__["_modules"]
        out = []
        for name in ("density_plane", "density_line", "app_plane", "app_line"):
            out.extend(d[1][name]._parameters.values())
        out.append(d[1]["basis_mat"]._parameters["weight"])
        out.append(d[1]["light_line"]._parameters["weight"])
        return out

    def packed_field(self) -> TirField:
        ps = self._field_params()
        mask = self.alphaMask
        key = (tuple((p.data_ptr(), p._version, tuple(p.shape)) for p in ps), id(mask),
               self.stepSize.data_ptr(), float(self.distance_scale), float(self.density_shift),
               float(self.rayMarch_weight_thres), float(self.near_far[0]), float(self.near_far[1]), self.fea2denseAct)
        if key == self._field_key and self._field_cache is not None:
            return self._field_cache["desc"]
        if len(set(self.density_n_comp)) != 1 or len(set(self.app_n_comp)) != 1:
            raise TensoirHipError("per-plane component counts must be equal for the gfx950 kernels")
        keep = {}
        f = TirField()
        g = _host_values(self, "geom", (self.aabb, self.invaabbSize, self.gridSize, self.stepSize),
                         lambda: (self.aabb[0].tolist(), self.aabb[1].tolist(), self.invaabbSize.tolist(),
                                  [int(v) for v in self.gridSize.tolist()], float(self.stepSize)))
        f.aabb_min[:], f.aabb_max[:], f.inv_aabb[:], f.grid[:], f.step_size = g
        f.distance_scale = float(self.distance_scale)
        f.density_shift = float(self.density_shift)
        f.weight_thres = float(self.rayMarch_weight_thres)
        f.near_, f.far_ = float(self.near_far[0]), float(self.near_far[1])
        f.act = {"softplus": 0, "relu": 1}[self.fea2denseAct]
        f.n_dcomp, f.n_acomp = self.density_n_comp[0], self.app_n_comp[0]
        f.app_dim, f.n_lights = self.app_dim, self.light_num
        for i in range(3):
            for name, src, dst in (("dp", self.density_plane, f.dplane), ("dl", self.density_line, f.dline),
                                   ("ap", self.app_plane, f.aplane), ("al", self.app_line, f.aline)):
                t = src[i].detach() if is_channel_last(src[i]) else ops.pack_plane(src[i])
                keep[f"{name}{i}"] = t
                dst[i] = t.data_ptr()
        keep["basis"] = ops.pack_basis(self.basis_mat.weight)
        keep["ll"] = self.light_line.weight.detach().to(torch.float32).contiguous()
        keep["lm"] = ops.light_mean(keep["ll"])
        f.basis_t, f.light_line, f.light_mean = keep["basis"].data_ptr(), keep["ll"].data_ptr(), keep["lm"].data_ptr()
        if mask is not None:
            keep["bits"] = mask.bits()
            f.occ_nbr = keep["bits"].data_ptr()
            D, H, W = mask.alpha_volume.shape[-3:]
            f.occ_dim[:] = [W, H, D]
            f.occ_aabb_min[:], f.occ_inv[:] = mask.host_geometry()
            lo, hi = mask.occupied_box()
            if all(a < b for a, b in zip(lo, hi)):
                f.occ_lo[:], f.occ_hi[:] = lo, hi
            else:
                f.occ_lo[:], f.occ_hi[:] = [3.0e38] * 3, [3.4e38] * 3
        f.tune_lds_lines, f.tune_xcd_order = ops.TUNE["lds_lines"], ops.TUNE["xcd_order"]
        keep["desc"] = f
        self._field_cache, self._field_key = keep, key
        return f

    def packed_field_half(self, _fresh=False):
        from ._lib import TirFieldHalf
        if not _fresh:
            self.packed_field()
        keep = self._field_cache
        if "half" not in keep:
            if self.app_n_comp[0] != 48:
                keep["half"] = None
            else:
                src = [keep[f"ap{i}"] for i in range(3)] + [keep[f"al{i}"] for i in range(3)]
                tabs, absmax = ops.pack_half(src, scan=(keep["ll"], keep["basis"]))
                fh = TirFieldHalf()
                for i in range(3):
                    fh.aplane[i], fh.aline[i] = tabs[i].data_ptr(), tabs[3 + i].data_ptr()
                keep["half"] = (fh, tabs)
                keep["half_range"] = ops.HalfRange(absmax)
        return keep["half"][0] if keep["half"] is not None else None

    def half_range(self, _fresh=False):
        return self._field_cache.get("half_range") if self.packed_field_half(_fresh) is not None else None

    def packed_field_dense(self, _fresh=False):
        if not _fresh:
            self.packed_field()
        keep = self._field_cache
        sel = (ops.TUNE["dense_sigma"], ops.TUNE["dense_sigma_max_mb"])
        ent = keep.get("dense")
        if ent is None or ent["sel"] != sel:
            if torch.cuda.is_current_stream_capturing():
                raise TensoirHipError("graph capture needs the dense density volume of the current field (run the pass eagerly first)")
            ent = keep["dense"] = self._build_dense(keep, sel)
        if ops.CAPTURE_KEEPALIVE is not None and ent["vol"] is not None:
            ops.CAPTURE_KEEPALIVE.append(ent["vol"])
        return ent["desc"]

    @staticmethod
    def _build_dense(keep, sel):
        f = keep["desc"]
        X, Y, Z = [int(g) for g in f.grid]
        nbytes = 4 * (X + 1) * Y * Z
        ent = {"sel": sel, "desc": f, "vol": None, "mb": nbytes / 2 ** 20, "why": None}
        if not sel[0]:
            ent["why"] = "switched off"
        elif nbytes > sel[1] * 2 ** 20:
            ent["why"] = "above the size cap"
        elif Y * Z >= 1 << 24 or 4 * (X + 1) >= 1 << 24 or nbytes >= 1 << 32:
            ent["why"] = "beyond 32-bit addressing"
        else:
            try:
                vol, pitch = ops.dense_sigma_build(f, keep["dp0"].device)
            except torch.cuda.OutOfMemoryError:
                ent["why"] = "allocation failed"
                return ent
            g = TirField.from_buffer_copy(f)
            g.dense_sigma, g.dense_pitch = vol.data_ptr(), pitch
            ent["desc"], ent["vol"] = g, vol
        return ent

    def dense_sigma_state(self):
        self.packed_field_dense()
        ent = self._field_cache["dense"]
        return {"on": ent["vol"] is not None, "why": ent["why"], "mb": ent["mb"]}

    def indirect_precision(self):
        return indirect.report(self)

    def compute_densityfeature(self, xyz_sampled):
        xyz = xyz_sampled.reshape(-1, 3)
        if _wants_grad("compute_densityfeature", xyz, *self._field_params()):
            from . import pointwise
            return pointwise.DensityFeatureFn.apply(self, xyz.detach(), *pointwise.density_params(self))
        return ops.vm_density(self.packed_field(), xyz)[0]

    def compute_densityfeature_with_xyz_grad(self, xyz_sampled):
        xyz = xyz_sampled.reshape(-1, 3)
        if _wants_grad("compute_densityfeature_with_xyz_grad", xyz, *self._field_params()):
            from . import pointwise
            return pointwise.DensityFeatXyzFn.apply(self, xyz, *pointwise.density_params(self))
        return ops.density_feat_grad(self.packed_field(), xyz, True, False)[0]

    def feature2density(self, density_features):
        if self.fea2denseAct == "softplus":
            return F.softplus(density_features + self.density_shift)
        return F.relu(density_features)

    def _app_features(self, what, xyz_sampled, light_idx, want_rad, want_int):
        xyz = xyz_sampled.reshape(-1, 3)
        li = light_idx.reshape(-1).to(xyz.device, torch.int32) if want_rad else None
        if _wants_grad(what, xyz, *self._field_params()):
            from . import pointwise
            return pointwise.AppFeatureFn.apply(self, xyz.detach(), li, want_rad, want_int, *pointwise.app_params(self))
        rad, intr = ops.vm_app(self.packed_field(), xyz, li, None, want_rad, want_int, ops.APP_IMPL)
        return tuple(t[:, :self.app_dim].contiguous() for t in (rad, intr) if t is not None)

    def compute_appfeature(self, xyz_sampled, light_idx):
        return self._app_features("compute_appfeature", xyz_sampled, light_idx, True, False)[0]

    def compute_bothfeature(self, xyz_sampled, light_idx):
        return self._app_features("compute_bothfeature", xyz_sampled, light_idx, True, True)

    def compute_intrinfeature(self, xyz_sampled):
        return self._app_features("compute_intrinfeature", xyz_sampled, None, False, True)[0]

    def compute_derived_normals(self, xyz_locs):
        xyz = xyz_locs.reshape(-1, 3)
        if _wants_grad("compute_derived_normals", xyz_locs, *self._field_params()):
            from . import pointwise
            xyz_locs.requires_grad_(True)
            return pointwise.DerivedNormalFn.apply(self, xyz_locs.reshape(-1, 3), *pointwise.density_params(self))
        return ops.density_grad(self.packed_field(), xyz)[2]

    def compute_alpha(self, xyz_locs, length=1):
        f = self.packed_field()
        xyz = xyz_locs.reshape(-1, 3).to(torch.float32)
        if _wants_grad("compute_alpha", xyz, *self._field_params()):
            from . import pointwise
            sigma = pointwise.DensitySigmaFn.apply(self, self.normalize_coord(xyz).detach(), *pointwise.density_params(self))
# ... 296 lines not shown
```

### tensoir_amd/graph.py

```python
from __future__ import annotations

import gc

import torch

from . import capacity, indirect, ops, relight
from ._lib import TensoirHipError
from .renderer import Renderer_TensoIR_train


class _OwnState:
    __slots__ = ("r", "saved")

    def __init__(self, renderer):
        self.r, self.saved = renderer, None

    def __enter__(self):
        d = self.r.model.__dict__
        self.saved = {k: d.pop(k) for k in GraphedRenderer._OWN_KEYS if k in d}
        d.update(self.r._own)

    def __exit__(self, *exc):
        d = self.r.model.__dict__
        self.r._own = {k: d.pop(k) for k in GraphedRenderer._OWN_KEYS if k in d}
        d.update(self.saved)
        self.saved = None


def _clone_grouped(out):
    bases, res = {}, {}
    for k, v in out.items():
        if not torch.is_tensor(v):
            res[k] = v
            continue
        st = v.untyped_storage()
        key = st.data_ptr()
        if key not in bases:
            nbytes = st.nbytes()
            if nbytes > 8 * v.numel() * v.element_size() + (1 << 16):
                bases[key] = None
            else:
                bases[key] = torch.empty(0, dtype=torch.uint8, device=v.device).set_(st, 0, (nbytes,), (1,)).clone()
        b = bases[key]
        res[k] = v.clone() if b is None else torch.empty(0, dtype=v.dtype, device=v.device).set_(
            b.untyped_storage(), v.storage_offset(), v.shape, v.stride())
    return res


class GraphedRenderer:
    def __init__(self, tensoIR, n_rays, N_samples=-1, white_bg=True, is_relight=True, sample_method="fixed_envirmap",
                 args=None, device="cuda"):
        if sample_method != "fixed_envirmap":
            raise TensoirHipError("GraphedRenderer supports sample_method='fixed_envirmap' only")
        self.model, self.n_rays, self.device = tensoIR, int(n_rays), torch.device(device)
        self.kw = dict(N_samples=N_samples, white_bg=white_bg, is_train=False, is_relight=is_relight,
                       sample_method=sample_method, chunk_size=160000, device=device, args=args)
        self.rays = torch.zeros((self.n_rays, 6), dtype=torch.float32, device=self.device)
        self.lidx = torch.zeros((self.n_rays, 1), dtype=torch.int32, device=self.device)
        self.graph = None
        self.out = None
        self.checks = []
        self._host = torch.zeros((9,), dtype=torch.int64).pin_memory()
        self._state = torch.zeros((5,), dtype=torch.int64, device=self.device)
        self._own = {}
        self._deferred = 0
        self.captures = 0
        self._model_key = None

    def _key(self):
        m = self.model
        m.packed_field()
        decs = [getattr(m, n) for n in ("renderModule", "renderModule_brdf", "renderModule_normal") if hasattr(m, n)]
        for d in decs:
            d.packed()
        lights = m.light_parameters()
        return (m._field_key, tuple((t.data_ptr(), t._version) for t in lights), tuple(d._key for d in decs),
                float(m.march_t_stop), ops.MLP_IMPL, ops.app_contraction(), ops.secondary_mlp_impl(), ops.secondary_app_impl(), ops.fused_indirect(),
                ops.INDIRECT_GUARD and indirect.verdict(m))

    def _stale(self):
        return self.graph is not None and self._key() != self._model_key

    _OWN_KEYS = ("_words", "_pair_counter", "_jit_rng")

    def _own_state(self):
        return _OwnState(self)

    def _eager(self):
        with torch.no_grad(), self._own_state():
            return Renderer_TensoIR_train(self.rays, None, self.lidx, self.model, _no_graph=True, **self.kw)

    def _capture(self):
        self._eager()
        self._eager()
        torch.cuda.synchronize()
        for key, cap in self.__dict__.get("_cap_floor", {}).items():
            hints, k, _ = capacity.check_site(self.model, key)
            if k in hints:
                hints[k] = max(hints[k], cap)
        shrink = self.__dict__.pop("_test_shrink_capacity", None)
        if shrink:
            for k in list(self.model._app_cap_hints):
                self.model._app_cap_hints[k] = shrink
        self.checks = []
        self.model.__dict__["_capture"] = self.checks
        self._keepalive = []
        g = torch.cuda.CUDAGraph()
        gc.collect()
        gc_was_on = gc.isenabled()
        gc.disable()
        try:
            ops.CAPTURE_KEEPALIVE = self._keepalive
            with torch.no_grad(), self._own_state(), torch.cuda.graph(g):
                self.out = Renderer_TensoIR_train(self.rays, None, self.lidx, self.model, _no_graph=True, **self.kw)
                if self.checks:
                    ops.record_check([t.reshape(1) for t, _, _ in self.checks], [c for _, c, _ in self.checks],
                                     self._state, self._host)
        finally:
            ops.CAPTURE_KEEPALIVE = None
            self.model.__dict__.pop("_capture", None)
            if gc_was_on:
                gc.enable()
        self.graph = g
        self._model_key = self._key()
        self.captures += 1
        if not shrink:
            floor = self.__dict__.setdefault("_cap_floor", {})
            for _, cap, key in self.checks:
                floor[key] = max(floor.get(key, 0), cap)

    def _overflowed(self):
        if not self.checks:
            return False
        torch.cuda.current_stream(self.device).synchronize()
        totals = self._host[:len(self.checks)].tolist()
        bad = False
        for total, (_, cap, key) in zip(totals, self.checks):
            if total > cap:
                bad = True
                self._need(key, total)
        return bad

    def _need(self, key, total):
        floor = self.__dict__.setdefault("_cap_floor", {})
        hints, k, need = capacity.check_site(self.model, key, total)
        floor[key] = max(floor.get(key, 0), need)
        hints.pop(k, None)

    def validate(self):
        torch.cuda.current_stream(self.device).synchronize()
        self._deferred = 0
        if int(self._host[8]) == 0:
            return True
        maxima = self._host[4:4 + len(self.checks)].tolist()
        for total, (_, cap, key) in zip(maxima, self.checks):
            if total > cap:
                self._need(key, total)
        self._clear_sticky()
        self.graph = None
        return False

# ... 31 lines not shown
```

### tensoir_amd/ops.py

```python
from __future__ import annotations

import ctypes as C
import math
import os

import numpy as np
import torch

from . import _lib
from ._lib import TirEnvSG, TirField, TirFieldHalf, TirMlp, check, lib

MAP_STRIDE = 20

STATS = None
TIMING = None

TUNE = {
    "lds_lines": 2 if os.environ.get("TENSOIR_LDS_LINES", "1") == "0" else 0,
    "xcd_order": 1 if os.environ.get("TIR_XCD", "0") == "1" else 0,
    "dense_sigma": 0 if os.environ.get("TENSOIR_DENSE_SIGMA", "1") == "0" else 1,
    "dense_sigma_max_mb": max(0, int(os.environ.get("TENSOIR_DENSE_SIGMA_MAX_MB", "1024") or 0)),
    "mlp_grid": max(0, int(os.environ.get("TENSOIR_MLP_GRID", "0") or 0)),
    "pair_order": 2 if os.environ.get("TIR_PAIR_ORDER", "d")[:1] == "m" else 0,
    "wgrad_blocks": max(0, int(os.environ.get("TENSOIR_WGRAD_BLOCKS", "0") or 0)),
}
AUX_TABLE = os.environ.get("TENSOIR_MLP_AUXTAB", "1") != "0"
AUX_TABLE_MULTI = os.environ.get("TENSOIR_MLP_AUXTAB_MULTI", "0") == "1"


def mlp_aux_table(m: "PackedMlp", aux):
    aux = f32(aux, "aux", 3)
    table = torch.empty((aux.shape[0], 128), dtype=torch.float32, device=aux.device)
    _call("tir_mlp_aux_table", C.byref(m.desc), _ptr(aux), aux.shape[0], _ptr(table), _stream())
    return table


CAPTURE_KEEPALIVE = None


def _aux_table_cached(m: "PackedMlp", aux):
    cache = m.__dict__.setdefault("_aux_tables", {})
    key = (aux.data_ptr(), aux._version, aux.shape[0])
    capturing = torch.cuda.is_current_stream_capturing()
    hit = cache.get(key)
    if hit is None:
        if capturing:
            return mlp_aux_table(m, aux)
        if len(cache) >= 4:
            cache.clear()
        table = mlp_aux_table(m, aux)
        ev = torch.cuda.Event()
        ev.record()
        hit = cache[key] = (aux, table, ev, _raw_stream(torch.cuda.current_device()) if _raw_stream else None)
    elif not capturing and (_raw_stream is None or hit[3] != _raw_stream(torch.cuda.current_device())):
        torch.cuda.current_stream().wait_event(hit[2])
    if capturing and CAPTURE_KEEPALIVE is not None:
        CAPTURE_KEEPALIVE.append(hit)
    return hit[1]


def mlp_rows_table(m: "PackedMlp", feat, table, n_dev=None, save_hidden=False):
    if MLP_IMPL != "bf16x3":
        raise NotImplementedError("per-row layer-1 tables exist for the split-bf16 decoder only (TENSOIR_MLP=bf16x3)")
    feat = f32(feat, "feat")
    n = feat.shape[0]
    table = f32(table, "table", 128)
    if table.shape[0] != n:
        raise ValueError("table must have one row per feature row")
    out = torch.empty((n, m.out_dim), dtype=torch.float32, device=feat.device)
    if not save_hidden:
        _call("tir_mlp_fwd_auxtab_bf16x3", C.byref(m.desc), _ptr(feat), feat.shape[1], _ptr(table), None, 0, _ptr(out), n,
              _ptr(n_dev), _stream())
        return out
    h1 = torch.empty((n, 128), dtype=torch.float32, device=feat.device)
    h2 = torch.empty((n, 128), dtype=torch.float32, device=feat.device)
    _call("tir_mlp_train_fwd_auxtab_bf16x3", C.byref(m.desc), _ptr(feat), feat.shape[1], _ptr(table), None, 0, _ptr(out),
          _ptr(h1), _ptr(h2), n, _ptr(n_dev), _stream())
    return out, h1, h2


def _stats_ptr(name, dev):
    if STATS is None:
        return None
    if name not in STATS:
        STATS[name] = torch.zeros((1,), dtype=torch.int64, device=dev)
    return C.c_void_p(STATS[name].data_ptr())


def _call(name, *args):
    with _timed(name):
        rc = getattr(lib(), name)(*args)
    check(rc, name)


class _timed:
    def __init__(self, name):
        self.name = name

    def __enter__(self):
        if TIMING is not None:
# ... 124 lines not shown
    tables = [t.detach() for t in tables]
    scan = [t.detach() for t in scan]
    for t in tables + scan:
        if t.dtype != torch.float32 or not t.is_cuda:
            raise ValueError("pack_half: fp32 CUDA tensors expected")
    outs = [torch.empty_strided(t.shape, t.stride(), dtype=torch.float16, device=t.device) for t in tables]
    k = len(tables) + len(scan)
    srcs = (C.c_void_p * k)(*[t.data_ptr() for t in tables + scan])
    dsts = (C.c_void_p * k)(*([o.data_ptr() for o in outs] + [None] * len(scan)))
    cnts = (C.c_int64 * k)(*[_storage_span(t) for t in tables + scan])
    absmax = torch.zeros((k,), dtype=torch.float32, device=(tables + scan)[0].device)
    _call("tir_pack_half_checked", srcs, dsts, cnts, k, _ptr(absmax), _stream())
    return outs, absmax


def _storage_span(t):
    n = 1 + sum((s - 1) * st for s, st in zip(t.shape, t.stride()))
    if n != t.numel():
        raise ValueError("pack_half: dense tensors expected")
    return n


def pack_occupancy(vol):
    vol = f32(vol.detach(), "alpha_volume")
    D, H, W = vol.shape[-3:]
    nbr = torch.empty(((D + 1) * (H + 1) * (W + 1),), dtype=torch.uint8, device=vol.device)
    _call("tir_pack_occupancy", _ptr(vol), _ptr(nbr), W, H, D, _stream())
    return nbr


def pack_basis(w):
    w = f32(w.detach(), "basis_mat.weight")
    app_dim, n_in = w.shape
    dst = torch.empty((n_in, 32), dtype=torch.float32, device=w.device)
    _call("tir_pack_basis", _ptr(w), _ptr(dst), app_dim, n_in, _stream())
    return dst


def light_mean(ll):
    ll = f32(ll.detach(), "light_line.weight")
    L, n = ll.shape
    out = torch.empty((n,), dtype=torch.float32, device=ll.device)
    _call("tir_light_mean", _ptr(ll), _ptr(out), L, n, _stream())
    return out


def pack_mlp(w0, b0, w1, b1, w2, b2, feat_dim, pe):
    ws = [f32(t.detach(), "mlp weight") for t in (w0, b0, w1, b1, w2, b2)]
    hidden, out_dim = w1.shape[0], w2.shape[0]
    n = lib().tir_mlp_packed_floats(feat_dim, pe, hidden, out_dim)
    if n < 0:
        check(int(n), f"tir_mlp_packed_floats(feat={feat_dim}, pe={pe}, hidden={hidden}, out={out_dim})")
    if tuple(w0.shape) != (hidden, feat_dim + 3 + 2 * pe * feat_dim + 2 * pe * 3):
        raise ValueError(f"mlp.0.weight has shape {tuple(w0.shape)}")
    packed = torch.empty((int(n),), dtype=torch.float32, device=w0.device)
    _call("tir_pack_mlp", *[_ptr(t) for t in ws], feat_dim, pe, hidden, out_dim, _ptr(packed),
                             _stream())
    return packed


class PackedMlp:
    def __init__(self, seq, feat_dim, pe, act, w0=None):
        self.packed = pack_mlp(seq[0].weight if w0 is None else w0, seq[0].bias, seq[2].weight, seq[2].bias,
                               seq[4].weight, seq[4].bias, feat_dim, pe)
        self.out_dim = seq[4].weight.shape[0]
        self.desc = TirMlp(self.packed.data_ptr(), feat_dim, pe, seq[2].weight.shape[0],
                           self.out_dim, act, TUNE["mlp_grid"])


def vm_density(field: TirField, xyz, want_feat=True, want_sigma=False):
    xyz = f32(xyz, "xyz", 3).view(-1, 3)
    n = xyz.shape[0]
    feat = torch.empty((n,), dtype=torch.float32, device=xyz.device) if want_feat else None
    sigma = torch.empty((n,), dtype=torch.float32, device=xyz.device) if want_sigma else None
    _call("tir_vm_density_fwd", C.byref(field), _ptr(xyz), _ptr(feat), _ptr(sigma), n, _stream())
    return feat, sigma


def dense_sigma_build(field: TirField, device):
    X, Y, Z = [int(g) for g in field.grid]
    pitch = X + 1
    vol = torch.empty((Z, Y, pitch), dtype=torch.float32, device=device)
    _call("tir_dense_sigma_build", C.byref(field), _ptr(vol), pitch, _stream())
    return vol, pitch


def dense_sigma(field: TirField, xyz, want_feat=True, want_sigma=False):
    xyz = f32(xyz, "xyz", 3).view(-1, 3)
    n = xyz.shape[0]
    feat = torch.empty((n,), dtype=torch.float32, device=xyz.device) if want_feat else None
    sigma = torch.empty((n,), dtype=torch.float32, device=xyz.device) if want_sigma else None
    _call("tir_dense_sigma_fwd", C.byref(field), _ptr(xyz), _ptr(feat), _ptr(sigma), n, _stream())
    return feat, sigma


def occupancy_query(field: TirField, xyz):
    xyz = f32(xyz, "xyz", 3).view(-1, 3)
    n = xyz.shape[0]
    hit = torch.empty((n,), dtype=torch.uint8, device=xyz.device)
    _call("tir_occupancy_query", C.byref(field), _ptr(xyz), _ptr(hit), n, _stream())
    return hit


def dense_alpha(field: TirField, grid_size, length):
    gx, gy, gz = [int(g) for g in grid_size]
    dev = torch.device("cuda", torch.cuda.current_device())
    lins = [torch.linspace(0, 1, g).to(dev).contiguous() for g in (gx, gy, gz)]
    alpha = torch.empty((gx, gy, gz), dtype=torch.float32, device=dev)
    _call("tir_dense_alpha", C.byref(field), _ptr(lins[0]), _ptr(lins[1]), _ptr(lins[2]), gx, gy, gz, float(length),
          _ptr(alpha), _stream())
    return alpha, lins


def alpha_pool(alpha, thres):
    alpha = f32(alpha, "alpha")
    gx, gy, gz = alpha.shape
    vol = torch.empty((gz, gy, gx), dtype=torch.float32, device=alpha.device)
    bbox = torch.tensor([2 ** 31 - 1] * 3 + [-1] * 3, dtype=torch.int32, device=alpha.device)
    _call("tir_alpha_pool", _ptr(alpha), gx, gy, gz, float(thres), _ptr(vol), _ptr(bbox), _stream())
    return vol, bbox


def filter_rays(field: TirField, rays, n_samples, bbox_only):
    rays = f32(rays, "rays", 6)
    n = rays.shape[0]
    mask = torch.empty((n,), dtype=torch.uint8, device=rays.device)
    _call("tir_filter_rays", C.byref(field), _ptr(rays), n, int(n_samples), int(bool(bbox_only)), _ptr(mask), _stream())
    return mask.bool()


def density_grad(field: TirField, xyz, want_sigma=False, want_grad=False, want_normal=True, n_dev=None):
    xyz = f32(xyz, "xyz", 3).view(-1, 3)
    n = xyz.shape[0]
    mk = lambda on, *s: torch.empty(s, dtype=torch.float32, device=xyz.device) if on else None
    sigma, grad, normal = mk(want_sigma, n), mk(want_grad, n, 3), mk(want_normal, n, 3)
    _call("tir_density_grad_fwd", C.byref(field), _ptr(xyz), _ptr(sigma), _ptr(grad), _ptr(normal),
                                     n, _ptr(n_dev), _stream())
    return sigma, grad, normal


FEAT_STRIDE = 32
APP_ENTRY = {"mfma": "tir_vm_app_fwd", "x3": "tir_vm_app_fwd_x3", "bf16x3": "tir_vm_app_fwd_bf16x3", "valu": "tir_vm_app_fwd_valu"}
APP_IMPL = os.environ.get("TENSOIR_APP", "mfma")


def vm_app(field: TirField, xyz, light_idx=None, idx_map=None, want_rad=True, want_int=False, impl=None,
           idx_div=0, n_dev=None):
    xyz = f32(xyz, "xyz", 3).view(-1, 3)
    n = xyz.shape[0]
    ad = FEAT_STRIDE
    if want_rad:
        if light_idx is None:
            raise ValueError("light_idx is required for the radiance feature")
        light_idx = i32(light_idx, "light_idx").view(-1)
        if idx_map is not None:
            idx_map = i32(idx_map, "idx_map").view(-1)
            if idx_map.numel() != n:
                raise ValueError("idx_map must have one entry per point")
        elif light_idx.numel() != n and idx_div <= 1:
            raise ValueError("light_idx must have one entry per point")
    rad = torch.empty((n, ad), dtype=torch.float32, device=xyz.device) if want_rad else None
    intr = torch.empty((n, ad), dtype=torch.float32, device=xyz.device) if want_int else None
    if impl is None:
        impl = "x3" if (APP_IMPL == "mfma" and app_contraction() == "x3" and int(field.n_acomp) in (16, 24, 48)) else APP_IMPL
    _call(APP_ENTRY[impl], C.byref(field), _ptr(xyz),
          _ptr(light_idx) if want_rad else None, _ptr(idx_map) if want_rad else None, _ptr(rad), _ptr(intr),
# ... 1694 lines not shown
```

### tensoir_amd/relight.py

```python
from __future__ import annotations

import functools
import os

import numpy as np
import torch

from . import capacity, indirect, ops
from .field_model import safe_l2_normalize

MAP_STRIDE = ops.MAP_STRIDE


_CONST_CACHE = {}


def _z_table(n_sample, near, far, device):
    key = ("z", int(n_sample), float(near), float(far), str(device))
    z = _CONST_CACHE.get(key)
    if z is None:
        t = torch.linspace(0.0, 1.0, n_sample, device=device)
        z = (near * (1.0 - t) + far * t).contiguous()
        _CONST_CACHE[key] = z
    return z
# ... 17 lines not shown
    if fh is not None and not full:
        feat = ops.vm_app_h16(f, fh, rec_xyz, light_idx, rec_ray, light_div, n_dev)
    else:
        feat = ops.vm_app(f, rec_xyz, light_idx, rec_ray, True, False, None, light_div, n_dev)[0]
    return ops.mlp(tensoIR.renderModule.packed(), feat, dirs, rec_ray if dir_map is None else
                   dir_map[rec_ray.long().clamp_(0, dir_map.numel() - 1)].contiguous(), None if full else ops.secondary_mlp_impl(),
                   n_dirs if dir_map is None else 0, n_dev)


def _fusable(f, dirs, dir_map, n_dirs, n_rows):
    return dir_map is None and n_dirs > 0 and dirs.shape[0] * 8 <= max(n_rows, 1) and int(f.app_dim) == 27 and int(f.n_acomp) == 48


def _decode_records(tensoIR, f, fh, kind, rec_xyz, rec_ray, n_dev, light_idx, light_div, dirs, dir_map, n_dirs):
    if _fusable(f, dirs, dir_map, n_dirs, rec_xyz.shape[0]):
        if kind == "f16" and fh is not None and ops.fused_indirect() and int(f.n_lights) <= 16:
            return ops.indirect_fused(f, fh, tensoIR.renderModule.packed(), rec_xyz, light_idx, rec_ray, light_div, dirs, n_dirs, n_dev)
        if kind == "hp" and ops.AUX_TABLE and ops.MLP_IMPL == "bf16x3" and int(f.n_lights) <= 8:
            return ops.indirect_fused_hp(f, tensoIR.renderModule.packed(), rec_xyz, light_idx, rec_ray, light_div, dirs, n_dirs, n_dev)
    return _gather_then_decode(tensoIR, f, fh, rec_xyz, light_idx, rec_ray, light_div, dirs, dir_map, n_dirs, n_dev, full=kind != "f16")


def _range_failed(tensoIR, rng):
    if rng is None or rng.ok():
        return False
    indirect.set_verdict(tensoIR, "full", "range", {"bound": rng.bound, "maxima": rng.maxima})
    return True


def _map_measure(probe_map, vis, packed, full_rows, count, n_rays, map_limit):
    def measure(cand):
        n_valid, ref = count(), full_rows()
        d = (cand[:n_valid] - ref[:n_valid]).double()
        delta = probe_map(vis, packed(cand), packed(ref))
        v = (torch.stack([d.mean(0).abs().max(), d.pow(2).mean().sqrt(), d.abs().max()]).tolist() if n_valid else [0.0, 0.0, 0.0])
        return delta <= map_limit, {"kind": "map", "map_max_abs": delta, "records": n_valid, "rays": n_rays, "bias": v[0], "rms": v[1],
                                    "max": v[2], "limit": map_limit}
    return measure


def _decode_pass(tensoIR, f, vis, rec, n_rows, n_dev, count, lookup, n_rays, force_full, keep_records, training, probe_map):
    capturing = tensoIR.__dict__.get("_capture") is not None
    mode = "full" if force_full else indirect.mode(tensoIR, training)
    if mode == "probe" and capturing:
        raise ops._lib.TensoirHipError("graph capture needs an established indirect-light precision verdict (run the pass eagerly first)")
    if n_rows <= 0:
        return torch.zeros((n_rays, 3), dtype=torch.float32, device=vis.device), None
    rec_ray, rec_w, rec_xyz = rec["ray"][:n_rows], rec["w"][:n_rows], rec["xyz"][:n_rows]
    fh = tensoIR.packed_field_half(_fresh=True) if (mode != "full" and ops.secondary_app_impl() == "h16") else None
    rng = tensoIR.half_range(_fresh=True) if (fh is not None and ops.INDIRECT_GUARD) else None
    if rng is not None and (mode == "probe" or rng.ready()):
        if _range_failed(tensoIR, rng):
            mode, fh = "full", None
        rng = None
    if capturing and rng is not None and not rng.ready():
        raise ops._lib.TensoirHipError("graph capture needs a finished range check of the fp16 field shadow (run the pass eagerly first)")

    def decode(kind):
        return _decode_records(tensoIR, f, fh, kind, rec_xyz, rec_ray, n_dev, *lookup)

    def packed(rgb):
        if keep_records:
            return {"off": rec["off"], "cnt": rec["cnt"], "w": rec_w, "rgb": rgb}
        return ops.accumulate_records(rec["off"], rec["cnt"], rec_w, rgb, n_rays)

    if mode != "probe":
        return packed(decode(mode)), rng
    if probe_map is not None:
        decode = functools.lru_cache(maxsize=None)(decode)
        measure = _map_measure(probe_map, vis, packed, lambda: decode("full"), lambda: min(count(), n_rows), n_rays,
                               ops.INDIRECT_PROBE["train_map_limit" if training else "map_limit"])
        try_hp = ops.INDIRECT_HP
    else:
        def measure(rows):
            return indirect.record_estimate(rows, min(count(), n_rows), lambda sel: _decode_records(
                tensoIR, f, None, "full", rec_xyz[sel].contiguous(), rec_ray[sel].contiguous(), None, *lookup))
        try_hp = ops.INDIRECT_HP and _fusable(f, *lookup[2:], n_rows) and ops.AUX_TABLE and ops.MLP_IMPL == "bf16x3"
    return packed(indirect.establish(tensoIR, decode, measure, try_hp, train_limit=training and probe_map is not None)[1]), rng


def _secondary(tensoIR, origins, dirs, n_rays, z, org_map, dir_map, active, light_idx, light_div,
               want_indirect, want_nerfactor=False, n_dirs=0, keep_records=False, ids=None, defer=False, training=False,
               probe_map=None):
    f = tensoIR.packed_field() if training else tensoIR.packed_field_dense()
    if not want_indirect:
        vis, oma, _ = ops.march_secondary(f, origins, dirs, z, n_rays, org_map, dir_map, active,
                                          tensoIR.march_t_stop, False, 0, want_nerfactor, n_dirs)
        return vis, oma, None
    rc = capacity.PassCapacity(tensoIR.__dict__.setdefault("_rec_cap_hints", {}), n_rays, 1.5, max_entries=32,
                               capture=tensoIR.__dict__.get("_capture"), check_key=("secondary", n_rays))
    first = rc.hinted() is None
    cap = _rec_capacity(n_rays) if first else rc.hinted()
    extra = {} if ids is None else dict(ray_ids=ids["pair_ids"], n_ids_dev=ids["n_active"], vis=ids["vis"], rec_cnt=ids["rec_cnt"])
    armed = tensoIR.__dict__.pop("_rec_counter_armed", None)
    if armed is not None and armed.device == origins.device:
        extra["counter"] = armed
    lookup, force_full = (light_idx, light_div, dirs, dir_map, n_dirs), False
    while True:
        vis, oma, rec = ops.march_secondary(f, origins, dirs, z, n_rays, org_map, dir_map, active,
                                            tensoIR.march_t_stop, True, cap, want_nerfactor, n_dirs, **extra)
        extra.pop("counter", None)
        n_total, n_dev = rec["counter"][0:1], rec["counter"][1:2]
        if first:
            total = int(n_total.item())
            if total > cap:
                cap = rc.regrow(total)
                continue
        else:
            rc.watch(n_total, cap)
        out, rng = _decode_pass(tensoIR, f, vis, rec, total if first else cap, n_dev, lambda: total if first else rc.count.get(), lookup,
                                n_rays, force_full, keep_records, training, probe_map)
        if not first and (defer or rc.capture is not None):
            break
        total = total if first else rc.count.get()
        if total <= cap and _range_failed(tensoIR, rng):
            force_full = True
        elif rc.settle(total):
            return vis, oma, out
        else:
            cap = rc.regrow(total)
    if rc.capture is None:
        tensoIR.__dict__.setdefault("_pending_checks", []).append(lambda: rc.settle() and not _range_failed(tensoIR, rng))
    elif _range_failed(tensoIR, rng):
        raise ops._lib.TensoirHipError("graph capture: the fp16 field shadow fails the range guard")
    return vis, oma, out


@torch.no_grad()
def compute_transmittance(tensoIR, surf_pts, light_in_dir, nSample=128, vis_near=0.1, vis_far=2, device="cuda"):
    surf_pts = surf_pts.to(torch.float32).contiguous()
    light_in_dir = light_in_dir.to(torch.float32).contiguous()
    z = _z_table(nSample, vis_near, vis_far, surf_pts.device)
    vis, oma, _ = _secondary(tensoIR, surf_pts, light_in_dir, surf_pts.shape[0], z, None, None, None,
                             None, 0, False, True)
    return vis, oma


@torch.no_grad()
def compute_radiance(tensoIR, surf_pts, light_in_dir, light_idx, nSample=128, vis_near=0.05, vis_far=1.5,
                     device=None):
    surf_pts = surf_pts.to(torch.float32).contiguous()
    light_in_dir = light_in_dir.to(torch.float32).contiguous()
    li = light_idx.reshape(-1).to(surf_pts.device, torch.int32).contiguous()
    z = _z_table(nSample, vis_near, vis_far, surf_pts.device)
    return _secondary(tensoIR, surf_pts, light_in_dir, surf_pts.shape[0], z, None, None, None, li, 0,
                      True, True)


@torch.no_grad()
def compute_secondary_shading_effects(tensoIR, surface_pts, surf2light, light_idx, nSample=96, vis_near=0.05,
                                      vis_far=1.5, chunk_size=15000, device="cuda"):
    vis, _, ind = compute_radiance(tensoIR, surface_pts, surf2light, light_idx, nSample, vis_near, vis_far)
    return vis.reshape(-1, 1), ind.reshape(-1, 3)


def GGX_specular(normal, pts2c, pts2l, roughness, fresnel):
    return ops.ggx_specular(normal, pts2c, pts2l, roughness, fresnel)


brdf_specular = GGX_specular


def linear2srgb_torch(tensor_0to1):
    if isinstance(tensor_0to1, np.ndarray):
        x = np.clip(tensor_0to1, 0, 1)
        return np.where(x <= 0.0031308, x * 12.92, 1.055 * np.power(x + 1e-6, 1 / 2.4) - (1.055 - 1))
    x = tensor_0to1.clamp(0, 1)
# ... 387 lines not shown
```

Measured before the change: 5.438 million.

## Precompute dense fp16 appearance-feature volume for indirect-light record decoding

Adds a build kernel that evaluates the VM appearance decomposition (plane×line×light products times the basis matrix) at every grid vertex and stores the 27 features as fp16 in a padded dense volume. Secondary-ray record decoding and the fp16 appearance path then do an 8-tap trilinear lookup of precomputed features, replacing per-sample plane/line gathers and the basis contraction. This trades extra memory and a one-time build per field for fewer loads and less arithmetic per sample. Results can drift slightly because features are quantized to fp16 at vertices and blended in fp16, and the path only applies to single-light 48-component, 27-feature fields.

```diff
diff --git a/include/tensoir_hip.h b/include/tensoir_hip.h
--- a/include/tensoir_hip.h
+++ b/include/tensoir_hip.h
@@ -46,6 +46,8 @@
     int32_t tune_xcd_order;
     const float* dense_sigma;
     int32_t dense_pitch;
+    int32_t dense_app_pitch;
+    const void* dense_app;
 } TirField;
 
 typedef struct TirFieldHalf {
@@ -101,6 +103,8 @@
 
 int tir_dense_sigma_build(const TirField* f, float* vol, int32_t pitch, void* stream);
 int tir_dense_sigma_fwd(const TirField* f, const float* xyz, float* feat, float* sigma, int64_t n, void* stream);
+
+int tir_dense_app_build(const TirField* f, void* vol, int32_t pitch, void* stream);
 
 int tir_density_grad_fwd(const TirField* f, const float* xyz, float* sigma, float* grad,
                          float* normal, int64_t n, const int32_t* n_dev, void* stream);
diff --git a/tensoir_amd/_lib.py b/tensoir_amd/_lib.py
--- a/tensoir_amd/_lib.py
+++ b/tensoir_amd/_lib.py
@@ -26,6 +26,7 @@
         ("occ_lo", C.c_float * 3), ("occ_hi", C.c_float * 3),
         ("tune_lds_lines", C.c_int32), ("tune_xcd_order", C.c_int32),
         ("dense_sigma", C.c_void_p), ("dense_pitch", C.c_int32),
+        ("dense_app_pitch", C.c_int32), ("dense_app", C.c_void_p),
     ]
 
 
@@ -69,6 +70,7 @@
     "tir_filter_rays": (C.c_int, [C.POINTER(TirField), P, I64, I32, I32, P, P]),
     "tir_dense_sigma_build": (C.c_int, [C.POINTER(TirField), P, I32, P]),
     "tir_dense_sigma_fwd": (C.c_int, [C.POINTER(TirField), P, P, P, I64, P]),
+    "tir_dense_app_build": (C.c_int, [C.POINTER(TirField), P, I32, P]),
     "tir_density_grad_fwd": (C.c_int, [C.POINTER(TirField), P, P, P, P, I64, P, P]),
     "tir_density_feat_grad_fwd": (C.c_int, [C.POINTER(TirField), P, P, P, I64, P]),
     "tir_vm_app_fwd": (C.c_int, [C.POINTER(TirField), P, P, P, P, P, I32, I32, I64, P, P]),
diff --git a/tensoir_amd/csrc/tir_common.hpp b/tensoir_amd/csrc/tir_common.hpp
--- a/tensoir_amd/csrc/tir_common.hpp
+++ b/tensoir_amd/csrc/tir_common.hpp
@@ -60,6 +60,18 @@
     if (!f->dense_sigma || f->dense_pitch <= f->grid[0]) return false;
     const int64_t Y = f->grid[1], Z = f->grid[2], pb = (int64_t)f->dense_pitch * 4;
     return f->grid[0] >= 2 && Y >= 1 && Z >= 1 && Y * Z < (1 << 24) && pb < (1 << 24) && Y * Z * pb < ((int64_t)1 << 32);
+}
+
+static inline bool tir_dense_app_index_ok(const int32_t (&grid)[3], int64_t pitch) {
+    const int64_t Y = grid[1], Z = grid[2], pb = pitch * 64;
+    return grid[0] >= 2 && Y >= 1 && Z >= 1 && Y * Z < (1 << 24) && pb < (1 << 24) && Y * Z * pb < ((int64_t)1 << 32);
+}
+
+static inline int tir_dense_app_route(const TirField* f) {
+    if (!f->dense_app) return f->dense_app_pitch ? TIR_ERR_ARG : 0;
+    if (f->dense_app_pitch <= f->grid[0] || reinterpret_cast<uintptr_t>(f->dense_app) % 16 != 0) return TIR_ERR_ARG;
+    if (!tir_dense_app_index_ok(f->grid, f->dense_app_pitch)) return TIR_ERR_UNSUPPORTED;
+    return f->n_lights == 1 && f->n_acomp == 48 && f->app_dim == 27 ? 1 : 0;
 }
 
 static inline bool tir_any_null(std::initializer_list<const void*> ptrs) {
@@ -580,6 +592,83 @@
     const float e = fmaf(b, ty.w.y, a * ty.w.x), g = fmaf(d, ty.w.y, c * ty.w.x);
     return fmaf(g, tz.w.y, e * tz.w.x);
 }
+
+__device__ __forceinline__ uint4 ld16b(const void* base, unsigned byte_off) {
+    return *reinterpret_cast<const uint4*>(reinterpret_cast<const char*>(base) + byte_off);
+}
+
+template <bool F32>
+__device__ __forceinline__ void dense_app_lookup(const TirField& f, float x, float y, float z, int h, float (&fo)[16]) {
+    const TapQ tx = make_tap_q(x, f.grid[0]), ty = make_tap_q(y, f.grid[1]), tz = make_tap_q(z, f.grid[2]);
+    const unsigned pb = (unsigned)f.dense_app_pitch * 64u, hb = 32u * (unsigned)h;
+    const unsigned xo[2] = {mad_u24(tx.i0, 64u, hb), mad_u24(tx.i1, 64u, hb)};
+    const unsigned z0 = mul_u24(tz.i0, (unsigned)f.grid[1]), z1 = mul_u24(tz.i1, (unsigned)f.grid[1]);
+    const unsigned row[4] = {z0 + ty.i0, z0 + ty.i1, z1 + ty.i0, z1 + ty.i1};
+    uint4 v[8][2];
+#pragma unroll
+    for (int c = 0; c < 8; ++c) {
+        const unsigned o = mad_u24(row[c >> 1], pb, xo[c & 1]);
+        v[c][0] = ld16b(f.dense_app, o);
+        v[c][1] = ld16b(f.dense_app, o + 16u);
+    }
+    const float wyz[4] = {tz.w.x * ty.w.x, tz.w.x * ty.w.y, tz.w.y * ty.w.x, tz.w.y * ty.w.y};
+    float w[8];
+#pragma unroll
+    for (int c = 0; c < 8; ++c) w[c] = wyz[c >> 1] * ((c & 1) ? tx.w.y : tx.w.x);
+    auto H = [](unsigned u) { return __builtin_bit_cast(tir_h2, u); };
+    if constexpr (F32) {
+#pragma unroll
+        for (int q = 0; q < 2; ++q)
+#pragma unroll
+            for (int p = 0; p < 4; ++p) {
+                float lo[2], hi[2];
+#pragma unroll
+                for (int g = 0; g < 2; ++g) {
+                    const unsigned u0[4] = {v[4 * g][q].x, v[4 * g][q].y, v[4 * g][q].z, v[4 * g][q].w};
+                    tir_h2 e = H(u0[p]);
+                    lo[g] = (float)e.x * w[4 * g]; hi[g] = (float)e.y * w[4 * g];
+#pragma unroll
+                    for (int c = 1; c < 4; ++c) {
+                        const unsigned uc[4] = {v[4 * g + c][q].x, v[4 * g + c][q].y, v[4 * g + c][q].z, v[4 * g + c][q].w};
+                        e = H(uc[p]);
+                        lo[g] = fmaf((float)e.x, w[4 * g + c], lo[g]); hi[g] = fmaf((float)e.y, w[4 * g + c], hi[g]);
+                    }
+                }
+                fo[8 * q + 2 * p] = lo[0] + lo[1];
+                fo[8 * q + 2 * p + 1] = hi[0] + hi[1];
+            }
+    } else {
+        tir_h2 hw[8];
+#pragma unroll
+        for (int c = 0; c < 8; ++c) hw[c] = tir_h2{(_Float16)w[c], (_Float16)w[c]};
+#pragma unroll
+        for (int q = 0; q < 2; ++q)
+#pragma unroll
+            for (int p = 0; p < 4; ++p) {
+                tir_h2 s[2];
+#pragma unroll
+                for (int g = 0; g < 2; ++g) {
+                    const unsigned u0[4] = {v[4 * g][q].x, v[4 * g][q].y, v[4 * g][q].z, v[4 * g][q].w};
+                    s[g] = H(u0[p]) * hw[4 * g];
+#pragma unroll
+                    for (int c = 1; c < 4; ++c) {
+                        const unsigned uc[4] = {v[4 * g + c][q].x, v[4 * g + c][q].y, v[4 * g + c][q].z, v[4 * g + c][q].w};
+                        s[g] = __builtin_elementwise_fma(H(uc[p]), hw[4 * g + c], s[g]);
+                    }
+                }
+                const tir_h2 r = s[0] + s[1];
+                fo[8 * q + 2 * p] = (float)r.x;
+                fo[8 * q + 2 * p + 1] = (float)r.y;
+            }
+    }
+}
+
+#ifndef TIR_DENSE_APP_F32
+#define TIR_DENSE_APP_F32 0
+#endif
+constexpr bool kDenseAppF32 = TIR_DENSE_APP_F32 != 0;
+constexpr int DA_CA = 48, DA_F = 27, DA_NF0 = 14;
+
 __device__ __forceinline__ unsigned lds_addr(const float* p) {
 #if defined(__HIP_DEVICE_COMPILE__)
     return (unsigned)(uintptr_t)(const __attribute__((address_space(3))) float*)p;
diff --git a/tensoir_amd/csrc/tir_dense_app.hip b/tensoir_amd/csrc/tir_dense_app.hip
--- /dev/null
+++ b/tensoir_amd/csrc/tir_dense_app.hip
@@ -0,0 +1,63 @@
+#include "tir_common.hpp"
+
+using namespace tir;
+
+__global__ void __launch_bounds__(256)
+k_dense_app_build(TirField f, uint4* __restrict__ vol, int pitch) {
+    __shared__ __attribute__((aligned(16))) float Bt[3 * DA_CA * 32];
+    __shared__ __attribute__((aligned(16))) float Lr[3 * DA_CA];
+    for (int i = threadIdx.x * 4; i < 3 * DA_CA * 32; i += 256 * 4) *reinterpret_cast<float4*>(Bt + i) = ld4(f.basis_t + i);
+    for (int i = threadIdx.x; i < 3 * DA_CA; i += 256) Lr[i] = f.light_line[i];
+    __syncthreads();
+    const int X = f.grid[0], Y = f.grid[1], Z = f.grid[2];
+    const int64_t i = (int64_t)blockIdx.x * blockDim.x + threadIdx.x;
+    if (i >= (int64_t)pitch * Y * Z) return;
+    const int x = (int)(i % pitch), y = (int)((i / pitch) % Y), z = (int)(i / ((int64_t)pitch * Y));
+    float acc[32];
+#pragma unroll
+    for (int j = 0; j < 32; ++j) acc[j] = 0.0f;
+    if (x < X) {
+        const float* const pl[3] = {f.aplane[0] + ((size_t)y * X + x) * DA_CA, f.aplane[1] + ((size_t)z * X + x) * DA_CA,
+                                    f.aplane[2] + ((size_t)z * Y + y) * DA_CA};
+        const float* const ln[3] = {f.aline[0] + (size_t)z * DA_CA, f.aline[1] + (size_t)y * DA_CA, f.aline[2] + (size_t)x * DA_CA};
+#pragma unroll 1
+        for (int k = 0; k < 3; ++k)
+#pragma unroll 1
+            for (int c = 0; c < DA_CA; c += 4) {
+                const float4 a = ld4(pl[k] + c), b = ld4(ln[k] + c), l = *reinterpret_cast<const float4*>(Lr + k * DA_CA + c);
+                const float p[4] = {(a.x * b.x) * l.x, (a.y * b.y) * l.y, (a.z * b.z) * l.z, (a.w * b.w) * l.w};
+#pragma unroll
+                for (int e = 0; e < 4; ++e) {
+                    const float* bt = Bt + (k * DA_CA + c + e) * 32;
+#pragma unroll
+                    for (int j = 0; j < 28; j += 4) {
+                        const float4 w = *reinterpret_cast<const float4*>(bt + j);
+                        acc[j] = fmaf(w.x, p[e], acc[j]); acc[j + 1] = fmaf(w.y, p[e], acc[j + 1]);
+                        acc[j + 2] = fmaf(w.z, p[e], acc[j + 2]); acc[j + 3] = fmaf(w.w, p[e], acc[j + 3]);
+                    }
+                }
+            }
+    }
+    unsigned pk[16];
+#pragma unroll
+    for (int h = 0; h < 2; ++h)
+#pragma unroll
+        for (int q = 0; q < 8; ++q) {
+            const int nf = h ? DA_F - DA_NF0 : DA_NF0, j0 = (h ? DA_NF0 : 0) + 2 * q;
+            const tir_h2 v = {2 * q < nf ? sat_half(acc[j0]) : (_Float16)0.0f, 2 * q + 1 < nf ? sat_half(acc[j0 + 1]) : (_Float16)0.0f};
+            pk[8 * h + q] = __builtin_bit_cast(unsigned, v);
+        }
+    uint4* o = vol + i * 4;
+#pragma unroll
+    for (int t = 0; t < 4; ++t) o[t] = make_uint4(pk[4 * t], pk[4 * t + 1], pk[4 * t + 2], pk[4 * t + 3]);
+}
+
+extern "C" int tir_dense_app_build(const TirField* f, void* vol, int32_t pitch, void* stream) {
+    if (!f) return TIR_ERR_ARG;
+    if (int rc = tir_check_app_field(f, TirAppNeeds().aligned().no_light_mean().width(DA_CA).app_dim_is(DA_F).no_feature_rows(), 0)) return rc;
+    if (!vol || pitch <= f->grid[0] || !tir_aligned16({vol, f->basis_t})) return TIR_ERR_ARG;
+    if (f->n_lights != 1 || !tir_dense_app_index_ok(f->grid, pitch)) return TIR_ERR_UNSUPPORTED;
+    const int64_t n = (int64_t)pitch * f->grid[1] * f->grid[2];
+    return tir_launch(k_dense_app_build, 0, dim3((unsigned)((n + 255) / 256)), dim3(256), 0, tir_stream(stream), *f,
+                      reinterpret_cast<uint4*>(vol), (int)pitch);
+}
diff --git a/tensoir_amd/csrc/tir_field.hip b/tensoir_amd/csrc/tir_field.hip
--- a/tensoir_amd/csrc/tir_field.hip
+++ b/tensoir_amd/csrc/tir_field.hip
@@ -1224,11 +1224,38 @@
     return pack_half_launch(srcs, dsts, counts, n_tables, absmax, stream);
 }
 
+__global__ void __launch_bounds__(256)
+k_vm_app_dense(TirField f, const float* __restrict__ xyz, float* __restrict__ rad_feat, int out_stride, int64_t n,
+               const int32_t* __restrict__ n_dev) {
+    if (n_dev) n = min(n, (int64_t)max(*n_dev, 0));
+    const int lane = threadIdx.x & 63, sl = lane & 31, h = lane >> 5;
+    const int64_t n_pass = (n + 31) / 32;
+    for (int64_t pass = (int64_t)blockIdx.x * 4 + (threadIdx.x >> 6); pass < n_pass; pass += (int64_t)gridDim.x * 4) {
+        const int64_t s = pass * 32 + sl, sc = s < n ? s : n - 1;
+        float fo[16];
+        dense_app_lookup<kDenseAppF32>(f, xyz[3 * sc], xyz[3 * sc + 1], xyz[3 * sc + 2], h, fo);
+        if (s >= n) continue;
+        float* o = rad_feat + s * out_stride + (h ? DA_NF0 : 0);
+        const int cols = h ? out_stride - DA_NF0 : DA_NF0;
+#pragma unroll
+        for (int r = 0; r < 16; ++r)
+            if (r < cols) o[r] = (h && r >= DA_F - DA_NF0) ? 0.0f : __builtin_amdgcn_fmed3f(fo[r], -65504.0f, 65504.0f);
+        for (int r = 16; r < cols; ++r) o[r] = 0.0f;
+    }
+}
+
 extern "C" int tir_vm_app_fwd_h16(const TirField* f, const TirFieldHalf* fh, const float* xyz, const int32_t* light_idx,
                                   const int32_t* idx_map, float* rad_feat, int32_t out_stride, int32_t idx_div, int64_t n,
                                   const int32_t* n_dev, void* stream) {
     if (!f || !fh) return TIR_ERR_ARG;
     if (int rc = tir_check_app_field(f, TirAppNeeds().fp16_tables(fh).aligned().element_index32().width(48), out_stride)) return rc;
+    const int dense = tir_dense_app_route(f);
+    if (dense < 0) return dense;
+    if (dense)
+        return tir_with_rows(n, {xyz, rad_feat, light_idx}, {}, [&] {
+            return tir_launch(k_vm_app_dense, 0, dim3(tir_gather_blocks(n, 128, 2048, 0)), dim3(256), 0, tir_stream(stream), *f, xyz,
+                              rad_feat, (int)out_stride, n, n_dev);
+        });
     return tir_with_rows(n, {xyz, rad_feat, light_idx}, {}, [&] {
         const int lt_rows = f->n_lights <= 16 ? f->n_lights : 0;
         const size_t lds = (size_t)(3 * 3 * 2 * 32) * 16 + (size_t)(lt_rows + 1) * 144 * sizeof(float) + (size_t)4 * 32 * TIR_XH * 2;
diff --git a/tensoir_amd/csrc/tir_mlp.hip b/tensoir_amd/csrc/tir_mlp.hip
--- a/tensoir_amd/csrc/tir_mlp.hip
+++ b/tensoir_amd/csrc/tir_mlp.hip
@@ -765,6 +765,86 @@
     c.e = ld_u4b(ln, g.l0 + o);  c.g = ld_u4b(ln, g.l1 + o);
 }
 
+template <bool PACK>
+__device__ __forceinline__ void fus_decode(const float* lds, unsigned w0hi, unsigned w1hi, const f32x16& facc, const float* __restrict__ table,
+                                           unsigned ai, int lane, int h, int64_t sd, int64_t n, float* __restrict__ out, int out_dim, int act) {
+    __builtin_amdgcn_s_setprio(FUS_DECODER_PRIO);
+    float fo[16];
+#pragma unroll
+    for (int r = 0; r < 16; ++r) fo[r] = __builtin_amdgcn_fmed3f(facc[r], -65504.0f, 65504.0f);
+    f32x16 acc[4];
+    if (PACK) {
+        const float* tp = table + (size_t)ai * HID + 4 * h;
+#pragma unroll
+        for (int mt = 0; mt < 4; ++mt)
+#pragma unroll
+            for (int i = 0; i < 4; ++i) {
+                const float4 t4 = *reinterpret_cast<const float4*>(tp + mt * 32 + 8 * i);
+                acc[mt][4 * i] = t4.x; acc[mt][4 * i + 1] = t4.y; acc[mt][4 * i + 2] = t4.z; acc[mt][4 * i + 3] = t4.w;
+            }
+    }
+    fus_layer1<0>(w0hi, fo, acc);
+    f32x16 acc2[4];
+    if constexpr (PACK) {
+        unsigned hp[32];
+#pragma unroll
+        for (int q = 0; q < 64; q += 2) {
+            const f32x2_t v2 = {acc[q >> 4][q & 15], acc[(q + 1) >> 4][(q + 1) & 15]};
+            fus_f16x2 hv = __builtin_convertvector(v2, fus_f16x2);
+            hv = __builtin_elementwise_min(__builtin_elementwise_max(hv, fus_f16x2{(_Float16)0.0f, (_Float16)0.0f}),
+                                           fus_f16x2{(_Float16)65504.0f, (_Float16)65504.0f});
+            hp[q >> 1] = __builtin_bit_cast(unsigned, hv);
+        }
+#pragma unroll
+        for (int mt = 0; mt < 4; ++mt) {
+            const float* bp = lds + BH_B1 + (h * 4 + mt) * 16;
+#pragma unroll
+            for (int r = 0; r < 16; ++r) acc2[mt][r] = bp[r];
+        }
+        fus_layer2p<0>(w1hi, hp, acc2);
+    } else {
+#pragma unroll
+        for (int mt = 0; mt < 4; ++mt) {
+            const float* bp = lds + BH_B1 + (h * 4 + mt) * 16;
+#pragma unroll
+            for (int r = 0; r < 16; ++r) acc2[mt][r] = bp[r];
+        }
+        layer2_interleaved<1, 0, true>(w1hi, w1hi, acc, acc2);
+    }
+    f32x4 o4[4];
+#pragma unroll
+    for (int c = 0; c < 4; ++c) o4[c] = f32x4{0.f, 0.f, 0.f, 0.f};
+    {
+        const float* wp = lds + BH_W2 + (h * 4 + (lane & 3)) * W2A_STRIDE;
+#pragma unroll
+        for (int g = 0; g < 16; ++g) {
+            const float4 w = *reinterpret_cast<const float4*>(wp + 4 * g);
+            const float wv[4] = {w.x, w.y, w.z, w.w};
+#pragma unroll
+            for (int e = 0; e < 4; ++e) {
+                const int q = 4 * g + e;
+                const float x = acc2[q >> 4][q & 15];
+                o4[e] = __builtin_amdgcn_mfma_f32_4x4x1f32(wv[e], x + __builtin_fabsf(x), o4[e], 0, 0, 0);
+            }
+        }
+    }
+    float o0 = (o4[0][0] + o4[1][0]) + (o4[2][0] + o4[3][0]);
+    float o1 = (o4[0][1] + o4[1][1]) + (o4[2][1] + o4[3][1]);
+    float o2 = (o4[0][2] + o4[1][2]) + (o4[2][2] + o4[3][2]);
+    float o3 = (o4[0][3] + o4[1][3]) + (o4[2][3] + o4[3][3]);
+    o0 += __shfl_xor(o0, 32, 64); o1 += __shfl_xor(o1, 32, 64);
+    o2 += __shfl_xor(o2, 32, 64); o3 += __shfl_xor(o3, 32, 64);
+    __builtin_amdgcn_s_setprio(0);
+    if (h == 0 && sd < n) {
+        const float* b2 = lds + BH_B2;
+        float* op = out + sd * out_dim;
+        op[0] = act_out(o0 + b2[0], act);
+        if (out_dim > 1) op[1] = act_out(o1 + b2[1], act);
+        if (out_dim > 2) op[2] = act_out(o2 + b2[2], act);
+        if (out_dim > 3) op[3] = act_out(o3 + b2[3], act);
+    }
+}
+
 template <int NW, bool PACK>
 __global__ void __launch_bounds__(NW * 64)
 k_indirect_fused(TirField f, TirFieldHalf fh, const float* __restrict__ packed, const float* __restrict__ xyz,
@@ -827,17 +907,6 @@
         f32x16 facc;
 #pragma unroll
         for (int r = 0; r < 16; ++r) facc[r] = 0.0f;
-        f32x16 acc[4];
-        auto load_table = [&]() {
-            const float* tp = table + (size_t)ai * HID + 4 * h;
-#pragma unroll
-            for (int mt = 0; mt < 4; ++mt)
-#pragma unroll
-                for (int i = 0; i < 4; ++i) {
-                    const float4 t4 = *reinterpret_cast<const float4*>(tp + mt * 32 + 8 * i);
-                    acc[mt][4 * i] = t4.x; acc[mt][4 * i + 1] = t4.y; acc[mt][4 * i + 2] = t4.z; acc[mt][4 * i + 3] = t4.w;
-                }
-        };
         {
             TapQ ax[3];
             unsigned xb[3][2];
@@ -873,71 +942,40 @@
                 __builtin_amdgcn_wave_barrier();
             }
         }
-        __builtin_amdgcn_s_setprio(FUS_DECODER_PRIO);
-        float fo[16];
-#pragma unroll
-        for (int r = 0; r < 16; ++r) fo[r] = __builtin_amdgcn_fmed3f(facc[r], -65504.0f, 65504.0f);
-        if (PACK) load_table();
-        fus_layer1<0>(w0hi, fo, acc);
-        f32x16 acc2[4];
-        if constexpr (PACK) {
-            unsigned hp[32];
-#pragma unroll
-            for (int q = 0; q < 64; q += 2) {
-                const f32x2_t v2 = {acc[q >> 4][q & 15], acc[(q + 1) >> 4][(q + 1) & 15]};
-                fus_f16x2 hv = __builtin_convertvector(v2, fus_f16x2);
-                hv = __builtin_elementwise_min(__builtin_elementwise_max(hv, fus_f16x2{(_Float16)0.0f, (_Float16)0.0f}),
-                                               fus_f16x2{(_Float16)65504.0f, (_Float16)65504.0f});
-                hp[q >> 1] = __builtin_bit_cast(unsigned, hv);
-            }
-#pragma unroll
-            for (int mt = 0; mt < 4; ++mt) {
-                const float* bp = lds + BH_B1 + (h * 4 + mt) * 16;
-#pragma unroll
-                for (int r = 0; r < 16; ++r) acc2[mt][r] = bp[r];
-            }
-            fus_layer2p<0>(w1hi, hp, acc2);
-        } else {
-#pragma unroll
-            for (int mt = 0; mt < 4; ++mt) {
-                const float* bp = lds + BH_B1 + (h * 4 + mt) * 16;
-#pragma unroll
-                for (int r = 0; r < 16; ++r) acc2[mt][r] = bp[r];
-            }
-            layer2_interleaved<1, 0, true>(w1hi, w1hi, acc, acc2);
-        }
-        f32x4 o4[4];
-#pragma unroll
-        for (int c = 0; c < 4; ++c) o4[c] = f32x4{0.f, 0.f, 0.f, 0.f};
-        {
-            const float* wp = lds + BH_W2 + (h * 4 + (lane & 3)) * W2A_STRIDE;
-#pragma unroll
-            for (int g = 0; g < 16; ++g) {
-                const float4 w = *reinterpret_cast<const float4*>(wp + 4 * g);
-                const float wv[4] = {w.x, w.y, w.z, w.w};
-#pragma unroll
-                for (int e = 0; e < 4; ++e) {
-                    const int q = 4 * g + e;
-                    const float x = acc2[q >> 4][q & 15];
-                    o4[e] = __builtin_amdgcn_mfma_f32_4x4x1f32(wv[e], x + __builtin_fabsf(x), o4[e], 0, 0, 0);
-                }
-            }
-        }
-        float o0 = (o4[0][0] + o4[1][0]) + (o4[2][0] + o4[3][0]);
-        float o1 = (o4[0][1] + o4[1][1]) + (o4[2][1] + o4[3][1]);
-        float o2 = (o4[0][2] + o4[1][2]) + (o4[2][2] + o4[3][2]);
-        float o3 = (o4[0][3] + o4[1][3]) + (o4[2][3] + o4[3][3]);
-        o0 += __shfl_xor(o0, 32, 64); o1 += __shfl_xor(o1, 32, 64);
-        o2 += __shfl_xor(o2, 32, 64); o3 += __shfl_xor(o3, 32, 64);
-        __builtin_amdgcn_s_setprio(0);
-        if (h == 0 && sd < n) {
-            const float* b2 = lds + BH_B2;
-            float* op = out + sd * out_dim;
-            op[0] = act_out(o0 + b2[0], act);
-            if (out_dim > 1) op[1] = act_out(o1 + b2[1], act);
-            if (out_dim > 2) op[2] = act_out(o2 + b2[2], act);
-            if (out_dim > 3) op[3] = act_out(o3 + b2[3], act);
-        }
+        fus_decode<PACK>(lds, w0hi, w1hi, facc, table, ai, lane, h, sd, n, out, out_dim, act);
+    }
+}
+
+template <int NW>
+__global__ void __launch_bounds__(NW * 64)
+k_indirect_fused_dense(TirField f, const float* __restrict__ packed, const float* __restrict__ xyz, const int32_t* __restrict__ rec_map,
+                       int aux_mod, const float* __restrict__ table, float* __restrict__ out, int64_t n,
+                       const int32_t* __restrict__ n_dev, int out_dim, int act) {
+    using namespace tir;
+    extern __shared__ __attribute__((aligned(16))) float lds[];
+    for (int i = threadIdx.x * 4; i < FH_FLOATS; i += NW * 64 * 4)
+        *reinterpret_cast<float4*>(lds + i) = *reinterpret_cast<const float4*>(packed + OFF_FF + i);
+    __syncthreads();
+    if (n_dev) n = min(n, (int64_t)max(*n_dev, 0));
+    const int lane = threadIdx.x & 63, wave = threadIdx.x >> 6;
+    const int sl = lane & 31, h = lane >> 5;
+    const unsigned lds0 = (unsigned)(size_t)lds;
+    const unsigned lane_off = lds0 + BH_FLOATS * 4 + (unsigned)(h * 128 + sl) * 16;
+    const unsigned w0hi = opaque(lane_off);
+    const unsigned w1hi = opaque(lane_off + BW0A_ELEMS * 2);
+    constexpr int TILE = NW * 32;
+    const int64_t n_tiles = (n + TILE - 1) / TILE;
+    const UDiv by_mod = make_udiv(aux_mod);
+    for (int64_t tile = blockIdx.x; tile < n_tiles; tile += gridDim.x) {
+        const int64_t sd = tile * TILE + wave * 32 + sl, sdc = sd < n ? sd : n - 1;
+        unsigned ai = rec_map ? (unsigned)rec_map[sdc] : (unsigned)sdc;
+        if (aux_mod > 0) udiv(ai, by_mod, ai);
+        float fr[16];
+        dense_app_lookup<kDenseAppF32>(f, xyz[3 * sdc], xyz[3 * sdc + 1], xyz[3 * sdc + 2], h, fr);
+        f32x16 facc;
+#pragma unroll
+        for (int r = 0; r < 16; ++r) facc[r] = fr[r];
+        fus_decode<true>(lds, w0hi, w1hi, facc, table, ai, lane, h, sd, n, out, out_dim, act);
     }
 }
 
@@ -2356,10 +2394,15 @@
     if (!f || !fh) return TIR_ERR_ARG;
     if (int rc = check_mlp(m)) return rc;
     if (int rc = tir_check_app_field(f, TirAppNeeds().fp16_tables(fh).aligned().element_index32().width(48).app_dim_is(F).no_feature_rows(), 0)) return rc;
+    const int dense = tir_dense_app_route(f);
+    if (dense < 0) return dense;
     return tir_with_rows(n, {xyz, light_idx, table, out}, {table}, [&] {
         if (!fused_index_ok(n, idx_div, aux_mod)) return (int)TIR_ERR_UNSUPPORTED;
         const int lt_rows = f->n_lights <= 16 ? f->n_lights : 0;
         constexpr int NW = 12; constexpr bool PACK = true;
+        if (dense)
+            return tir_launch(k_indirect_fused_dense<NW>, FH_BYTES, dim3(decoder_grid(n, NW * 32, m->tune_grid)), dim3(NW * 64), FH_BYTES,
+                              tir_stream(stream), *f, m->packed, xyz, rec_map, aux_mod, table, out, n, n_dev, m->out_dim, m->act);
         const size_t lds = (size_t)FH_BYTES + FUS_WH_BYTES + (size_t)(lt_rows + 1) * 144 * sizeof(float) + (size_t)NW * 32 * FUS_XH * 2;
         return tir_launch(k_indirect_fused<NW, PACK>, (int)lds, dim3(decoder_grid(n, NW * 32, m->tune_grid)), dim3(NW * 64), lds,
                           tir_stream(stream), *f, *fh, m->packed, xyz, light_idx, rec_map, idx_div, aux_mod, table, out, n, n_dev,
diff --git a/tensoir_amd/field_model.py b/tensoir_amd/field_model.py
--- a/tensoir_amd/field_model.py
+++ b/tensoir_amd/field_model.py
@@ -574,7 +574,7 @@
     def half_range(self, _fresh=False):
         return self._field_cache.get("half_range") if self.packed_field_half(_fresh) is not None else None
 
-    def packed_field_dense(self, _fresh=False):
+    def packed_field_dense(self, _fresh=False, app=False):
         if not _fresh:
             self.packed_field()
         keep = self._field_cache
@@ -586,7 +586,53 @@
             ent = keep["dense"] = self._build_dense(keep, sel)
         if ops.CAPTURE_KEEPALIVE is not None and ent["vol"] is not None:
             ops.CAPTURE_KEEPALIVE.append(ent["vol"])
-        return ent["desc"]
+        if not app:
+            return ent["desc"]
+        asel = (ops.TUNE["dense_app"], ops.TUNE["dense_app_max_mb"])
+        aent = ent.get("app")
+        if aent is None or aent["sel"] != asel:
+            if torch.cuda.is_current_stream_capturing():
+                raise TensoirHipError("graph capture needs the dense appearance volume of the current field (run the pass eagerly first)")
+            aent = ent["app"] = self._build_dense_app(keep, ent, asel)
+        if ops.CAPTURE_KEEPALIVE is not None and aent["vol"] is not None:
+            ops.CAPTURE_KEEPALIVE.append(aent["vol"])
+        return aent["desc"]
+
+    @staticmethod
+    def _build_dense_app(keep, ent, sel):
+        f = ent["desc"]
+        nbytes = ops.dense_app_bytes(f)
+        X, Y, Z = [int(g) for g in f.grid]
+        aent = {"sel": sel, "desc": f, "vol": None, "mb": nbytes / 2 ** 20, "why": None}
+        if not sel[0]:
+            aent["why"] = "switched off"
+        elif ent["vol"] is None:
+            aent["why"] = "no dense density volume"
+        elif int(f.n_lights) != 1:
+            aent["why"] = "several lights"
+        elif int(f.n_acomp) != 48 or int(f.app_dim) != 27:
+            aent["why"] = "not a 48-component, 27-feature field"
+        elif nbytes > sel[1] * 2 ** 20:
+            aent["why"] = "above the size cap"
+        elif Y * Z >= 1 << 24 or 64 * (X + 1) >= 1 << 24 or nbytes >= 1 << 32:
+            aent["why"] = "beyond 32-bit addressing"
+        else:
+            try:
+                vol, pitch = ops.dense_app_build(f, keep["ap0"].device)
+            except torch.cuda.OutOfMemoryError:
+                aent["why"] = "allocation failed"
+                return aent
+            g = TirField.from_buffer_copy(f)
+            g.dense_app, g.dense_app_pitch = vol.data_ptr(), pitch
+            aent["desc"], aent["vol"] = g, vol
+        return aent
+
+    def dense_app_state(self, training=False):
+        if training:
+            return {"on": False, "why": "training pass", "mb": ops.dense_app_bytes(self.packed_field()) / 2 ** 20}
+        self.packed_field_dense(app=True)
+        aent = self._field_cache["dense"]["app"]
+        return {"on": aent["vol"] is not None, "why": aent["why"], "mb": aent["mb"]}
 
     @staticmethod
     def _build_dense(keep, sel):
diff --git a/tensoir_amd/graph.py b/tensoir_amd/graph.py
--- a/tensoir_amd/graph.py
+++ b/tensoir_amd/graph.py
@@ -76,7 +76,8 @@
         lights = m.light_parameters()
         return (m._field_key, tuple((t.data_ptr(), t._version) for t in lights), tuple(d._key for d in decs),
                 float(m.march_t_stop), ops.MLP_IMPL, ops.app_contraction(), ops.secondary_mlp_impl(), ops.secondary_app_impl(), ops.fused_indirect(),
-                ops.INDIRECT_GUARD and indirect.verdict(m))
+                ops.INDIRECT_GUARD and indirect.verdict(m),
+                ops.TUNE["dense_sigma"], ops.TUNE["dense_sigma_max_mb"], ops.TUNE["dense_app"], ops.TUNE["dense_app_max_mb"])
 
     def _stale(self):
         return self.graph is not None and self._key() != self._model_key
diff --git a/tensoir_amd/ops.py b/tensoir_amd/ops.py
--- a/tensoir_amd/ops.py
+++ b/tensoir_amd/ops.py
@@ -16,6 +16,8 @@
 TIMING = None
 
 TUNE = {
+    "dense_app": 0 if os.environ.get("TENSOIR_DENSE_APP", "1") == "0" else 1,
+    "dense_app_max_mb": max(0, int(os.environ.get("TENSOIR_DENSE_APP_MAX_MB", "4096") or 0)),
     "lds_lines": 2 if os.environ.get("TENSOIR_LDS_LINES", "1") == "0" else 0,
     "xcd_order": 1 if os.environ.get("TIR_XCD", "0") == "1" else 0,
     "dense_sigma": 0 if os.environ.get("TENSOIR_DENSE_SIGMA", "1") == "0" else 1,
@@ -306,6 +308,19 @@
     pitch = X + 1
     vol = torch.empty((Z, Y, pitch), dtype=torch.float32, device=device)
     _call("tir_dense_sigma_build", C.byref(field), _ptr(vol), pitch, _stream())
+    return vol, pitch
+
+
+def dense_app_bytes(field: TirField):
+    X, Y, Z = [int(g) for g in field.grid]
+    return 64 * (X + 1) * Y * Z
+
+
+def dense_app_build(field: TirField, device):
+    X, Y, Z = [int(g) for g in field.grid]
+    pitch = X + 1
+    vol = torch.empty((Z, Y, pitch, 2, 16), dtype=torch.float16, device=device)
+    _call("tir_dense_app_build", C.byref(field), _ptr(vol), pitch, _stream())
     return vol, pitch
 
 
diff --git a/tensoir_amd/relight.py b/tensoir_amd/relight.py
--- a/tensoir_amd/relight.py
+++ b/tensoir_amd/relight.py
@@ -123,7 +123,7 @@
 def _secondary(tensoIR, origins, dirs, n_rays, z, org_map, dir_map, active, light_idx, light_div,
                want_indirect, want_nerfactor=False, n_dirs=0, keep_records=False, ids=None, defer=False, training=False,
                probe_map=None):
-    f = tensoIR.packed_field() if training else tensoIR.packed_field_dense()
+    f = tensoIR.packed_field() if training else tensoIR.packed_field_dense(app=bool(want_indirect))
     if not want_indirect:
         vis, oma, _ = ops.march_secondary(f, origins, dirs, z, n_rays, org_map, dir_map, active,
                                           tensoIR.march_t_stop, False, 0, want_nerfactor, n_dirs)
```

After: 6.014 million, median of 6. 1.11x the previous value.
